# kcat/openal-soft

Hardware: AMD Instinct MI355X
Metric: mixed voices/sec @48kHz 1024-sample update, HRTF stereo; fraction of HBM roofline (higher is better)
Workload: dtype f32

## Files before the change

include/oalgpu.h:

```cpp
#ifndef OALGPU_H
#define OALGPU_H

#include <stddef.h>
#include <stdint.h>

#ifdef __cplusplus
extern "C" {
#endif
#if defined(__GNUC__)
#pragma GCC visibility push(default)
#endif

#define OALGPU_BUFFER_LINE_SIZE 1024
#define OALGPU_MAX_RESAMPLER_PADDING 48
#define OALGPU_MAX_RESAMPLER_EDGE 24
#define OALGPU_HRTF_HISTORY_LENGTH 64
#define OALGPU_HRIR_LENGTH 128
#define OALGPU_MAX_SENDS 6
#define OALGPU_MAX_OUTPUT_CHANNELS 32
#define OALGPU_MAX_AMBI_CHANNELS 25
#define OALGPU_MIXER_FRAC_BITS 16

typedef enum oalgpu_error {
    OALGPU_OK = 0,
// ... 24 lines not shown
    OALGPU_BIQUAD_HIGHSHELF, OALGPU_BIQUAD_LOWSHELF, OALGPU_BIQUAD_PEAKING, OALGPU_BIQUAD_LOWPASS,
    OALGPU_BIQUAD_HIGHPASS, OALGPU_BIQUAD_BANDPASS
} oalgpu_biquad_type;

typedef enum oalgpu_math_mode { OALGPU_MATH_EXACT = 0, OALGPU_MATH_FAST = 1 } oalgpu_math_mode;

const char *oalgpu_version(void);
const char *oalgpu_last_error(void);
int oalgpu_device_count(void);

typedef struct oalgpu_bsinc_table {
    float scaleBase, scaleRange;
    uint32_t m[16];
    uint32_t filterOffset[16];
    const float *tab;
    size_t tablen;
} oalgpu_bsinc_table;
int oalgpu_bsinc_table_get(int which , oalgpu_bsinc_table *out);
int oalgpu_cubic_table_get(int which , float *out);

typedef struct oalgpu_interp_state {
    int32_t kind;
    int32_t table;
    float sf;
    uint32_t m, l;
    uint32_t filter_offset;
} oalgpu_interp_state;
int oalgpu_prepare_resampler(int resampler, uint32_t increment, oalgpu_interp_state *out);

typedef struct oalgpu_biquad {
    float z1, z2;
    float b0, b1, b2, a1, a2;
    float tb0, tb1, tb2, ta1, ta2;
    int32_t counter;
} oalgpu_biquad;
void oalgpu_biquad_reset(oalgpu_biquad *f);
void oalgpu_biquad_set_params_from_slope(oalgpu_biquad *f, int type, float f0norm, float gain,
    float slope);

int oalgpu_resample(int device, int mode, int resampler, uint32_t increment, const float *src,
    size_t srclen, uint32_t frac, float *dst, size_t n);
int oalgpu_mix(int device, const float *in, size_t n, float *out, size_t nlines,
    float *current_gains, const float *target_gains, size_t counter, size_t outpos);
int oalgpu_mix_hrtf(int device, int mode, const float *in, float *accum, uint32_t irsize,
    const float *coeffs, const uint32_t delay[2], float gain, float gainstep, size_t n);
int oalgpu_mix_hrtf_blend(int device, int mode, const float *in, float *accum, uint32_t irsize,
    const float *oldcoeffs, const uint32_t olddelay[2], float oldgain, const float *newcoeffs,
    const uint32_t newdelay[2], float newgainstep, size_t n);
typedef struct oalgpu_splitter { float coeff, lp_z1, lp_z2, ap_z1; } oalgpu_splitter;
void oalgpu_splitter_init(oalgpu_splitter *s, float f0norm);
int oalgpu_mix_direct_hrtf(int device, int mode, float *left, float *right, const float *in,
    size_t nch, float *accum, oalgpu_splitter *splitters, const float *hfscales,
    const float *chan_coeffs, size_t irsize, size_t n);
int oalgpu_biquad_dual_process(int device, oalgpu_biquad *f0, oalgpu_biquad *f1, const float *src,
    float *dst, size_t n);

typedef struct oalgpu_context oalgpu_context;

typedef struct oalgpu_context_desc {
    int32_t  device;
    int32_t  math_mode;
    uint32_t sample_rate;
    uint32_t num_dry_channels;
    uint32_t num_real_channels;
    uint32_t num_aux_sends;
    uint32_t num_slots;
    uint32_t wet_channels;
    int32_t  hrtf;
    uint32_t max_voices;
    uint32_t max_buffers;
    uint32_t voices_per_group;
    uint32_t flags;
} oalgpu_context_desc;
#define OALGPU_CTX_FIR_VALU 1u
#define OALGPU_CTX_PROFILE  2u
#define OALGPU_CTX_STREAM_ROWS 8u
#define OALGPU_CTX_APPLY_IN_VOICE_KERNEL 16u
#define OALGPU_CTX_FUSED_REDUCE 32u
#define OALGPU_CTX_RESIDENT 64u
#define OALGPU_CTX_SLICE_LINES 128u
#define OALGPU_CTX_WAVE_PAIRS 256u
#define OALGPU_CTX_ROW_SLICES 512u
#define OALGPU_CTX_SERIAL   4u

int  oalgpu_context_create(const oalgpu_context_desc *desc, oalgpu_context **out);
void oalgpu_context_destroy(oalgpu_context *ctx);

int oalgpu_hrtf_load_mhr(oalgpu_context *ctx, const void *data, size_t size);
int oalgpu_hrtf_load_store(oalgpu_context *ctx, uint32_t sample_rate, uint32_t ir_size, const float *field_distance,
    const uint8_t *field_evcount, uint32_t num_fields, const uint16_t *elev_azcount, const uint16_t *elev_iroffset,
    uint32_t num_elevs, const float *coeffs, const uint8_t *delays, uint32_t num_irs);
typedef struct oalgpu_hrtf_info {
    uint32_t sample_rate, ir_size, num_fields, num_elevs, num_irs;
} oalgpu_hrtf_info;
int oalgpu_hrtf_info_get(oalgpu_context *ctx, oalgpu_hrtf_info *out);
int oalgpu_hrtf_raw(oalgpu_context *ctx, float *field_distance, uint8_t *field_evcount,
    uint16_t *elev_azcount, uint16_t *elev_iroffset, float *coeffs, uint8_t *delays);
int oalgpu_hrtf_get_coeffs(oalgpu_context *ctx, const float *dirs, size_t count, float *coeffs,
    uint32_t *delays);
int oalgpu_set_direct_hrtf(oalgpu_context *ctx, const float *chan_coeffs ,
    const float *hfscales, float xover_norm, uint32_t irsize);
int oalgpu_set_direct_hrtf_from_store(oalgpu_context *ctx, const float *points, const float *matrix, uint32_t num_points,
    const float *order_hf_gain, float xover_freq, uint32_t ir_size, int per_hrir_min);
int oalgpu_hrtf_parse_host(const void *mhr, size_t size, uint32_t device_rate, oalgpu_hrtf_info *info, float *coeffs, uint8_t *delays);
int oalgpu_hrtf_blend_host(const void *mhr, size_t size, uint32_t device_rate, const float *dirs, size_t count,
    uint32_t *idx, float *w, float *pass, uint32_t *delays);
int oalgpu_hrtf_build_direct_host(const void *mhr, size_t size, uint32_t device_rate, uint32_t ir_size, int per_hrir_min,
    const float *points, const float *matrix, uint32_t num_points, uint32_t num_chans, float xover_freq, const float *order_hf_gain,
    float *out_coeffs, float *out_hfscales, float *out_xover_norm, uint32_t *out_irsize);

int oalgpu_buffer_register(oalgpu_context *ctx, const void *data, int fmt_type,
    uint32_t frame_step, uint32_t sample_len, uint32_t loop_start, uint32_t loop_end);
int oalgpu_buffer_release(oalgpu_context *ctx, int buffer);
int oalgpu_buffer_info(oalgpu_context *ctx, int buffer, int32_t *live, int32_t *release_pending, uint32_t *references);

int oalgpu_buffer_channel_view(oalgpu_context *ctx, int buffer, uint32_t channel);

typedef struct oalgpu_voice_desc {
    int32_t  buffer;
    int32_t  looping;
    int32_t  position;
    uint32_t position_frac;
    uint32_t frequency;
} oalgpu_voice_desc;
int oalgpu_voice_init(oalgpu_context *ctx, uint32_t voice, const oalgpu_voice_desc *desc);
int oalgpu_context_set_nfc(oalgpu_context *ctx, float w1, const uint32_t channels_per_order[5]);
int oalgpu_voice_set_nfc(oalgpu_context *ctx, uint32_t voice, float w0);

int oalgpu_voice_set_ambi_scale(oalgpu_context *ctx, uint32_t voice, float xover_norm, float hf_scale,
    float lf_scale);

typedef struct oalgpu_filter_params {
    int32_t active;
    float gain_hf, hf_norm;
    float gain_lf, lf_norm;
} oalgpu_filter_params;

typedef struct oalgpu_voice_params {
    uint32_t step;
    int32_t  resampler;
    oalgpu_filter_params direct_filter;
    float    dry_gains[OALGPU_MAX_OUTPUT_CHANNELS];
    float    hrtf_ev, hrtf_az, hrtf_dist, hrtf_spread;
    float    hrtf_gain;
    int32_t  send_slot[OALGPU_MAX_SENDS];
    oalgpu_filter_params send_filter[OALGPU_MAX_SENDS];
    float    send_gains[OALGPU_MAX_SENDS][OALGPU_MAX_AMBI_CHANNELS];
} oalgpu_voice_params;
#define OALGPU_HRTF_KEEP_TARGET (-1.0f)
int oalgpu_voice_set_hrtf_targets(oalgpu_context *ctx, const uint32_t *voices, const float *coeffs, const uint32_t *delays,
    const float *gains, size_t count);

typedef struct oalgpu_voice_pan {
    float dir[3];
    float spread;
    float dry_gain;
    float send_gain[OALGPU_MAX_SENDS];
} oalgpu_voice_pan;
int oalgpu_context_set_ambi_map(oalgpu_context *ctx, const uint8_t *index, const float *scale);
int oalgpu_slot_set_ambi_map(oalgpu_context *ctx, uint32_t slot, const uint8_t *index, const float *scale);
int oalgpu_voice_set_pan(oalgpu_context *ctx, const uint32_t *voices, const oalgpu_voice_pan *pans, size_t count);

int oalgpu_buffer_queue_link(oalgpu_context *ctx, int buffer, int next_buffer);
int oalgpu_voice_init_queue(oalgpu_context *ctx, uint32_t voice, int first_buffer, int looping, int32_t position,
    uint32_t position_frac);
int oalgpu_voice_queue_state(oalgpu_context *ctx, uint32_t voice, int32_t *current_buffer, uint32_t *buffers_done);
// ... 182 lines not shown
    oalgpu_biquad direct_lp, direct_hp;
    float    send_current[OALGPU_MAX_SENDS][OALGPU_MAX_AMBI_CHANNELS];
    oalgpu_biquad send_lp[OALGPU_MAX_SENDS], send_hp[OALGPU_MAX_SENDS];
} oalgpu_voice_state;
int oalgpu_voice_readback(oalgpu_context *ctx, uint32_t voice, oalgpu_voice_state *out);
typedef struct oalgpu_voice_brief {
    int32_t  play_state;
    int32_t  position;
    uint32_t position_frac;
    int32_t  has_buffer;
    int32_t  fading;
    int32_t  current_buffer;
    uint32_t buffers_done;
} oalgpu_voice_brief;
int oalgpu_voices_readback(oalgpu_context *ctx, const uint32_t *voices, size_t count, oalgpu_voice_brief *out);

typedef struct oalgpu_voice_move {
    uint32_t voice;
    float hrtf_ev, hrtf_az, hrtf_dist, hrtf_spread;
    float hrtf_gain;
} oalgpu_voice_move;
int oalgpu_voice_move_async(oalgpu_context *ctx, const oalgpu_voice_move *moves, size_t count);
int oalgpu_read_output_async(oalgpu_context *ctx, uint32_t *ticket);
int oalgpu_output_wait(oalgpu_context *ctx, uint32_t ticket, float *out, size_t out_floats);

typedef struct oalgpu_voice_event {
    uint32_t voice;
    int32_t  play_state;
    int32_t  has_buffer;
    int32_t  current_buffer;
    uint32_t buffers_done;
    int32_t  position;
    uint32_t position_frac;
    int32_t  fading;
} oalgpu_voice_event;
int oalgpu_voice_events_async(oalgpu_context *ctx, uint32_t *ticket);
int oalgpu_voice_events_wait(oalgpu_context *ctx, uint32_t ticket, oalgpu_voice_event *out, size_t capacity, size_t *count);

int oalgpu_last_update_ms(oalgpu_context *ctx, float *total_ms, float *voice_kernel_ms);
int oalgpu_set_timing(oalgpu_context *ctx, int enable);
enum oalgpu_effect_kind {
    OALGPU_EFFECT_EQUALIZER = 0, OALGPU_EFFECT_MODULATOR, OALGPU_EFFECT_ECHO, OALGPU_EFFECT_DEDICATED, OALGPU_EFFECT_COMPRESSOR,
    OALGPU_EFFECT_CHORUS, OALGPU_EFFECT_DISTORTION, OALGPU_EFFECT_AUTOWAH, OALGPU_EFFECT_VMORPHER, OALGPU_EFFECT_FSHIFTER,
    OALGPU_EFFECT_PSHIFTER
};
enum oalgpu_modulator_waveform { OALGPU_MODULATOR_SINUSOID = 0, OALGPU_MODULATOR_SAWTOOTH, OALGPU_MODULATOR_SQUARE };
#define OALGPU_INVALID_CHANNEL 0xffffffffu
typedef struct oalgpu_equalizer_props {
    float low_cutoff, low_gain, mid1_center, mid1_gain, mid1_width, mid2_center, mid2_gain, mid2_width, high_cutoff, high_gain;
} oalgpu_equalizer_props;
typedef struct oalgpu_modulator_props { float frequency, high_pass_cutoff; int32_t waveform; } oalgpu_modulator_props;
typedef struct oalgpu_echo_props { float delay, lr_delay, damping, feedback, spread; } oalgpu_echo_props;
typedef struct oalgpu_compressor_props { int32_t on_off; } oalgpu_compressor_props;
enum oalgpu_chorus_waveform { OALGPU_CHORUS_SINUSOID = 0, OALGPU_CHORUS_TRIANGLE };
enum oalgpu_vmorpher_waveform { OALGPU_VMORPHER_SINUSOID = 0, OALGPU_VMORPHER_TRIANGLE, OALGPU_VMORPHER_SAWTOOTH };
enum oalgpu_fshifter_direction { OALGPU_FSHIFTER_DOWN = 0, OALGPU_FSHIFTER_UP, OALGPU_FSHIFTER_OFF };
typedef struct oalgpu_chorus_props { int32_t waveform, phase; float rate, depth, feedback, delay; } oalgpu_chorus_props;
typedef struct oalgpu_distortion_props { float edge, gain, lowpass_cutoff, eq_center, eq_bandwidth; } oalgpu_distortion_props;
typedef struct oalgpu_autowah_props { float attack_time, release_time, resonance, peak_gain; } oalgpu_autowah_props;
typedef struct oalgpu_vmorpher_props {
    float rate; int32_t phoneme_a, phoneme_b, phoneme_a_coarse_tuning, phoneme_b_coarse_tuning, waveform;
} oalgpu_vmorpher_props;
typedef struct oalgpu_fshifter_props { float frequency; int32_t left_direction, right_direction; } oalgpu_fshifter_props;
typedef struct oalgpu_pshifter_props { int32_t coarse_tune, fine_tune; } oalgpu_pshifter_props;
typedef struct oalgpu_effect oalgpu_effect;
int  oalgpu_effect_create(int device, int math_mode, int kind, uint32_t sample_rate, uint32_t num_in_channels,
    uint32_t num_out_lines, oalgpu_effect **out);
void oalgpu_effect_destroy(oalgpu_effect *effect);
int  oalgpu_effect_update(oalgpu_effect *effect, const void *props, const uint32_t *target_channels, const float *gains);
int  oalgpu_effect_process(oalgpu_effect *effect, const float *wet_in, float *out_lines, uint32_t n);
int  oalgpu_effect_set_upsampler(oalgpu_effect *effect, const float order_scales[2], float xover_norm);
int  oalgpu_slot_set_effect(oalgpu_context *ctx, uint32_t slot, oalgpu_effect *effect);

typedef struct oalgpu_converter oalgpu_converter;
int  oalgpu_converter_create(int device, int src_type, int dst_type, uint32_t channels, uint32_t src_rate,
    uint32_t dst_rate, int resampler, oalgpu_converter **out);
void oalgpu_converter_destroy(oalgpu_converter *conv);
uint32_t oalgpu_converter_available_out(const oalgpu_converter *conv, uint32_t src_frames);
int  oalgpu_converter_convert(oalgpu_converter *conv, const void **src, uint32_t *src_frames, void *dst,
    uint32_t dst_frames);

const char *oalgpu_voice_kernel_name(oalgpu_context *ctx);

typedef struct oalgpu_convolution oalgpu_convolution;
int  oalgpu_convolution_create(int device, uint32_t num_out_lines, const float *ir, uint32_t ir_len,
    oalgpu_convolution **out);
int  oalgpu_convolution_create_ex(int device, uint32_t num_out_lines, const float *ir, uint32_t ir_frames,
    uint32_t channels, uint32_t ir_rate, uint32_t device_rate, oalgpu_convolution **out);
void oalgpu_convolution_destroy(oalgpu_convolution *conv);
int  oalgpu_polyphase_resample(uint32_t src_rate, uint32_t dst_rate, const double *in, size_t n_in, double *out,
    size_t n_out);
int  oalgpu_convolution_set_target_gains(oalgpu_convolution *conv, const float *gains);
int  oalgpu_convolution_set_channel_gains(oalgpu_convolution *conv, const float *gains);
int  oalgpu_convolution_set_upsample(oalgpu_convolution *conv, const float *hf_scales, const float *lf_scales,
    float xover_norm);
int  oalgpu_convolution_process(oalgpu_convolution *conv, const float *wet_in, float *out_lines, uint32_t n);
int  oalgpu_convolution_process_device(oalgpu_convolution *conv, void *hip_stream, const float *wet_in_dev,
    float *out_lines_dev, uint32_t n);
int  oalgpu_slot_set_convolution(oalgpu_context *ctx, uint32_t slot, oalgpu_convolution *conv);

typedef struct oalgpu_reverb_props {
    float density, diffusion, gain, gain_hf, gain_lf, decay_time, decay_hf_ratio, decay_lf_ratio;
    float reflections_gain, reflections_delay, reflections_pan[3];
    float late_reverb_gain, late_reverb_delay, late_reverb_pan[3];
    float echo_time, echo_depth, modulation_time, modulation_depth, air_absorption_gain_hf;
    float hf_reference, lf_reference, room_rolloff_factor;
    int32_t decay_hf_limit;
} oalgpu_reverb_props;

typedef struct oalgpu_bq_coeffs { float b0, b1, b2, a1, a2; } oalgpu_bq_coeffs;
typedef struct oalgpu_reverb_pipeline {
    oalgpu_bq_coeffs filter_lp, filter_hp;
    uint32_t early_delay_tap[4][2];
    float    early_delay_coeff[2];
    uint32_t late_delay_tap[4][2];
    float    mix_x, mix_y;
    float    early_ap_coeff;
    uint32_t early_ap_offset[4];
    uint32_t early_offset[4];
    float    early_coeff;
    float    early_gains_target[4][OALGPU_MAX_AMBI_CHANNELS];
    uint32_t late_offset[4];
    float    late_density_gain;
    float    t60_mid_gain[4];
    oalgpu_bq_coeffs t60_hf[4], t60_lf[4];
    uint32_t mod_step;
    float    mod_depth;
    float    late_ap_coeff;
    uint32_t late_ap_offset[4];
    float    late_gains_target[4][OALGPU_MAX_AMBI_CHANNELS];
    uint32_t fade_sample_count;
} oalgpu_reverb_pipeline;
typedef struct oalgpu_reverb_params {
    int32_t pipeline_state;
    int32_t current_pipeline;
    oalgpu_reverb_pipeline pipe[2];
} oalgpu_reverb_params;
enum oalgpu_reverb_pipeline_state {
    OALGPU_REVERB_DEVICE_CLEAR = 0, OALGPU_REVERB_START_FADE = 1, OALGPU_REVERB_FADING = 2,
    OALGPU_REVERB_CLEANUP = 3, OALGPU_REVERB_NORMAL = 4
};

typedef struct oalgpu_reverb oalgpu_reverb;
int  oalgpu_reverb_create(int device, uint32_t sample_rate, uint32_t num_out_lines, oalgpu_reverb **out);
void oalgpu_reverb_destroy(oalgpu_reverb *rev);
int  oalgpu_reverb_set_upmix(oalgpu_reverb *rev, const float order_scales[2], const float *first_order_up,
    float xover_norm);
int  oalgpu_reverb_set_stream(oalgpu_reverb *rev, void *hip_stream);
int  oalgpu_reverb_set_math_mode(oalgpu_reverb *rev, int math_mode);
int  oalgpu_reverb_update(oalgpu_reverb *rev, const oalgpu_reverb_props *props, float slot_gain);
int  oalgpu_reverb_get_params(oalgpu_reverb *rev, oalgpu_reverb_params *out);
int  oalgpu_reverb_set_params(oalgpu_reverb *rev, const oalgpu_reverb_params *params);
int  oalgpu_reverb_line_lengths(oalgpu_reverb *rev, uint32_t lengths[11]);
int  oalgpu_reverb_process(oalgpu_reverb *rev, const float *wet_in, float *out_lines, uint32_t n);
int  oalgpu_reverb_process_device(oalgpu_reverb *rev, const float *wet_in_dev, float *out_lines_dev, uint32_t n);
int  oalgpu_reverb_skip(oalgpu_reverb *rev, uint32_t n);
int  oalgpu_slot_set_reverb(oalgpu_context *ctx, uint32_t slot, oalgpu_reverb *rev);

int  oalgpu_slot_set_target(oalgpu_context *ctx, uint32_t slot, int32_t target_slot);
int  oalgpu_slot_target(oalgpu_context *ctx, uint32_t slot, int32_t *target_slot);
int  oalgpu_slot_order(const int32_t *targets, uint32_t num_slots, uint32_t *order, uint32_t *depth);

#if defined(__GNUC__)
#pragma GCC visibility pop
#endif
#ifdef __cplusplus
// ... 4 lines not shown
```

openal-soft_amd/csrc/api.hip:

```cpp
#include "api_context.hpp"
namespace oalgpu {

thread_local std::string gLastError;

int Fail(int code, const std::string &msg)
{
    gLastError = msg;
    return code;
}

int UseDevice(int device)
{
    int count = 0;
    if(hipGetDeviceCount(&count) != hipSuccess || count <= 0)
        return Fail(OALGPU_ERR_NO_DEVICE, "no HIP device available (the product has no CPU path)");
    if(device < 0 || device >= count) return Fail(OALGPU_ERR_INVALID, "device ordinal out of range");
    HIP_TRY(hipSetDevice(device));
    ParkResidentContexts(device);
    return OALGPU_OK;
}

}

int UseCtx(oalgpu_context *c)
// ... 143 lines not shown
    L.firMfma = (desc->flags & OALGPU_CTX_FIR_VALU) ? 0u : 1u;
    c->serialOnly = (desc->flags & OALGPU_CTX_SERIAL) != 0;
    c->res.enabled = (desc->flags & OALGPU_CTX_RESIDENT) != 0 && !(desc->flags & (OALGPU_CTX_PROFILE | OALGPU_CTX_SERIAL));
    c->useWave = WaveKernelApplies(c->exact, L);
    if(c->useWave)
    {
        L.waveVoices = desc->voices_per_group ? std::max<uint32_t>(1u, (desc->voices_per_group + 3u) / 4u)
            : std::max<uint32_t>(1u, (desc->max_voices + 2047u) / 2048u);
        L.numGroups = std::max<uint32_t>(1u, WaveKernelGroups(L));
    }
    const TableBlob &blob = Blob();
    HIP_TRY(c->tables.alloc(blob.data.size())); HIP_TRY(c->tables.upload(blob.data.data(), blob.data.size()));
    L.tables = c->tables.p;
    HIP_TRY(c->buffers.alloc(std::max<uint32_t>(desc->max_buffers, 1u))); HIP_TRY(c->buffers.zero());
    L.buffers = c->buffers.p;
    c->buf.reset(desc->max_buffers, desc->max_voices);
    c->cbOfVoice.assign(std::max<uint32_t>(desc->max_voices, 1u), -1);

    const size_t nv = desc->max_voices;
    HIP_TRY(c->ctl.alloc(nv)); HIP_TRY(c->ctl.zero()); L.ctl = c->ctl.p;
    HIP_TRY(c->prev.alloc(nv * kMaxPad)); HIP_TRY(c->prev.zero()); L.prev = c->prev.p;
    HIP_TRY(c->dfilt.alloc(nv * 2)); HIP_TRY(c->dfilt.zero()); L.dfilt = c->dfilt.p;
    HIP_TRY(c->hist.alloc(nv * kHist)); HIP_TRY(c->hist.zero()); L.hist = c->hist.p;
    HIP_TRY(c->gainCur.alloc(nv * L.numDry)); HIP_TRY(c->gainCur.zero()); L.gainCur = c->gainCur.p;
    HIP_TRY(c->gainTgt.alloc(nv * L.numDry)); HIP_TRY(c->gainTgt.zero()); L.gainTgt = c->gainTgt.p;
    HIP_TRY(c->sfilt.alloc(nv * L.numSends * 2)); HIP_TRY(c->sfilt.zero()); L.sfilt = c->sfilt.p;
    HIP_TRY(c->sendCur.alloc(nv * L.numSends * L.wetChannels)); HIP_TRY(c->sendCur.zero()); L.sendCur = c->sendCur.p;
    HIP_TRY(c->sendTgt.alloc(nv * L.numSends * L.wetChannels)); HIP_TRY(c->sendTgt.zero()); L.sendTgt = c->sendTgt.p;
    HIP_TRY(c->ambi.alloc(nv)); HIP_TRY(c->ambi.zero()); L.ambi = c->ambi.p;
    HIP_TRY(c->startDelay.alloc(nv)); HIP_TRY(c->startDelay.zero()); L.startDelay = c->startDelay.p;
    {
        std::vector<AmbiMapEntry> ident(std::max<size_t>(L.numDry, size_t{L.numSlots} * L.wetChannels) + 1);
        for(size_t i = 0; i < ident.size(); ++i) ident[i] = AmbiMapEntry{uint32_t(i < OALGPU_MAX_AMBI_CHANNELS ? i : 0), 1.0f};
        HIP_TRY(c->dryMap.alloc(L.numDry)); HIP_TRY(c->dryMap.upload(ident.data(), L.numDry));
        HIP_TRY(c->wetMaps.alloc(size_t{L.numSlots} * L.wetChannels));
        for(uint32_t s = 0; s < L.numSlots; ++s)
            HIP_TRY(hipMemcpy(c->wetMaps.p + size_t{s} * L.wetChannels, ident.data(), L.wetChannels * sizeof(AmbiMapEntry), hipMemcpyHostToDevice));
    }
    HIP_TRY(c->queueDone.alloc(nv)); HIP_TRY(c->queueDone.zero()); L.queueDone = c->queueDone.p;
    L.numLineGroups = L.numGroups;
    c->groupsAllocated = L.numGroups;
    if(c->useWave && L.hrtf && L.firMfma && !(desc->flags & OALGPU_CTX_WAVE_PAIRS))
    {
        const uint32_t w = Wave16WavesFor(desc->max_voices, DeviceComputeUnits(desc->device));
        c->groupsAllocated = std::max<uint32_t>(c->groupsAllocated, (desc->max_voices + w - 1u) / w);
    }
    L.streams = nullptr; L.lineGains = nullptr; L.lineStride = 0; L.streamsPerVoice = 0;
    L.nfc = nullptr; L.nfcOrders = 0;
    L.hrirs = nullptr;
    for(uint32_t &n : L.chansPerOrder) n = 0;
    L.accLines = 0;
    L.wave16 = 0;
    L.rows8 = 0; L.rowsVpg = 0;
    if(c->useWave && !(desc->flags & OALGPU_CTX_STREAM_ROWS))
    {
        L.accLines = WaveKernelAccLines(L);
        if(!L.accLines && RowsKernelApplies(L))
            L.rows8 = 1;
    }
    if(c->useWave && (!L.hrtf || L.numSends))
    {
        L.lineStride = L.mixLines <= 8 ? 8u : (L.mixLines <= 16 ? 16u : 32u);
        L.streamsPerVoice = 2u + L.numSends;
    }
    if(c->useWave && (!L.hrtf || L.numSends) && !L.accLines && !L.rows8) { if(int rc = AllocStreamRows(c.get())) return rc; }
    const size_t groups = c->groupsAllocated;
    HIP_TRY(c->partLines.alloc(groups * L.mixLines * kLine)); L.partLines = c->partLines.p;
    HIP_TRY(c->partLines2.alloc(c->useWave && (L.streams || L.accLines || L.rows8) ? groups * L.mixLines * kLine : 0));
    c->partLinesBuf[0] = c->partLines.p; c->partLinesBuf[1] = c->partLines2.p;
    HIP_TRY(c->partHrtf.alloc(L.hrtf ? groups * (kLine + kHrirLen) * 2 : 0)); L.partHrtf = c->partHrtf.p;
    HIP_TRY(c->partHrtf2.alloc(c->useWave && L.hrtf ? groups * (kLine + kHrirLen) * 2 : 0));
    c->partHrtfBuf[0] = c->partHrtf.p; c->partHrtfBuf[1] = c->partHrtf2.p;
    HIP_TRY(c->bus.alloc(BusFloats(L))); HIP_TRY(c->bus.zero()); L.bus = c->bus.p;
    if(desc->flags & OALGPU_CTX_PROFILE)
    {
        HIP_TRY(c->phaseTimes.alloc(nv * 16)); HIP_TRY(c->phaseTimes.zero());
        c->prof.times = c->phaseTimes.p;
    }
    L.hrtfOld = nullptr; L.hrtfTgt = nullptr;

    HIP_TRY(c->dSplit.alloc(L.numDry)); HIP_TRY(c->dSplit.zero());
    HIP_TRY(c->dSplit2.alloc(L.numDry)); HIP_TRY(c->dSplit2.zero());
    HIP_TRY(c->carryBuf.alloc(size_t{kLine + kHrirLen} * 2)); HIP_TRY(c->carryBuf.zero());
    HIP_TRY(c->postArrived.alloc(1)); HIP_TRY(c->postArrived.zero());
    HIP_TRY(c->dHfScale.alloc(L.numDry)); HIP_TRY(c->dHfScale.zero());
    HIP_TRY(c->dCoeffs.alloc(size_t{L.numDry} * kHrirLen * 2)); HIP_TRY(c->dCoeffs.zero());
    HIP_TRY(c->dTemp.alloc(size_t{L.numDry} * kLine + (kLine + kHrirLen) * 2));
    if(L.rows8) SetRowsGroups(c.get());
    *out = c.release();
    return OALGPU_OK;
}

void oalgpu_context_destroy(oalgpu_context *ctx)
{
    if(!ctx) return;
    (void)UseDevice(ctx->desc.device);
    if(ctx->attachedTo || !ctx->attached.empty()) DetachForDestroy(ctx);
    if(ctx->res.pendingBlock) { ctx->res.pendingBlock->heldBy = nullptr; ctx->res.pendingBlock = nullptr; }
    (void)FlushPendingMix(ctx);
    (void)hipStreamSynchronize(ctx->stream);
    if(ctx->res.reduceStream) (void)hipStreamSynchronize(ctx->res.reduceStream);
    if(ctx->postStream) (void)hipStreamSynchronize(ctx->postStream);
    delete ctx->comm;
    for(auto &cb : ctx->cbVoices)
        for(int k = 0; k < 2; ++k)
        {
            if(cb.pinned[k]) (void)hipHostFree(cb.pinned[k]);
            if(cb.copied[k]) (void)hipEventDestroy(cb.copied[k]);
        }
    delete ctx;
}

int AllocStreamRows(oalgpu_context *c)
{
    DeviceLayout &L = c->L;
    const size_t nv = L.numVoices;
    HIP_TRY(c->streams.alloc(nv * L.streamsPerVoice * kLine)); HIP_TRY(c->streams.zero()); L.streams = c->streams.p;
    HIP_TRY(c->lineGains.alloc(nv * L.streamsPerVoice * LineBlockDwords(L.lineStride))); HIP_TRY(c->lineGains.zero());
    L.lineGains = c->lineGains.p;
    return OALGPU_OK;
}

const float *CarrySource(oalgpu_context *c, bool carry)
{
    const float *src = nullptr;
    if(carry && c->L.hrtf) src = c->carryInBuf ? c->carryBuf.p : c->L.bus + BusAccumOffset(c->L);
    c->carryInBuf = false;
    return src;
}

static void SplitterRunPowers(float coeff, uint32_t seg, float out[4])
{
    const float ap = coeff, lp = coeff * 0.5f + 0.5f;
    float st[3][3] = {{1.0f, 0.0f, 0.0f}, {0.0f, 1.0f, 0.0f}, {0.0f, 0.0f, 1.0f}};
    for(uint32_t i = 0; i < seg; ++i)
        for(auto &v : st)
        {
            const float d0 = (0.0f - v[0]) * lp;
            const float lpY0 = v[0] + d0;
            v[0] = std::fmaf(d0, lp, lpY0);
            const float d1 = (lpY0 - v[1]) * lp;
            const float lpY1 = v[1] + d1;
            v[1] = lpY1 + d1;
            const float apY = std::fmaf(0.0f, ap, v[2]);
            v[2] = std::fmaf(-apY, ap, 0.0f);
        }
    out[0] = st[0][0]; out[1] = st[0][1]; out[2] = st[1][1]; out[3] = st[2][2];
}

int PostDirectHrtfFused(oalgpu_context *c, hipStream_t s, uint32_t samples_to_do, hipEvent_t evDone, bool resident)
{
    const DeviceLayout &L = c->L;
    float *left = L.bus + size_t{L.numDry} * kLine;
    SplitterState *spIn = c->dSplitCur ? c->dSplit2.p : c->dSplit.p, *spOut = c->dSplitCur ? c->dSplit.p : c->dSplit2.p;
    const uint32_t postEpoch = c->postEpoch + L.numDry;
    const uint32_t seg = ((samples_to_do + 63u) / 64u) | 1u;
    if(c->runPowerSeg != seg) { SplitterRunPowers(c->dSplitCoeff, seg, c->runPower); c->runPowerSeg = seg; }
    const uint32_t slot = c->outNext % oalgpu_context::kIoSlots;
    const bool ring = c->outRing && c->outFlags;
    const uint32_t outTarget = c->outArrivedTotal + PostResidentFirGroups();
    const PostHrtfCall call{left, left + kLine, L.bus, L.numDry, L.bus + BusAccumOffset(L), c->carryBuf.p, spIn, spOut, c->dHfScale.p, c->dCoeffs.p,
        c->dIrSize, samples_to_do, c->dTemp.p, c->postArrived.p, postEpoch, c->runPower, evDone, ring ? c->outHost[slot] : nullptr,
        ring ? c->outFlags + size_t{slot} * 16 : nullptr, c->outSeq + 1u};
    auto &R = c->res;
    if(resident)
    {
        c->reduceHeld = false;
        LaunchPostResident(s, call, R.counters.p, R.hostFlags, (R.posts + 1u) * R.redGroups, (R.posts + 1u) * R.firGroups, R.posts + 1u);
        HIP_TRY(hipGetLastError());
        ++R.posts;
    }
    else if(c->reduceHeld)
    {
        c->reduceHeld = false;
        if(!c->reducedCount.p) { HIP_TRY(c->reducedCount.alloc(1)); HIP_TRY(c->reducedCount.zero()); }
        const uint32_t reducedEpoch = c->reducedEpoch + ReducePostReduceGroups(c->heldL);
        LaunchReducePostFused(s, call, c->heldL, CarrySource(c, c->carryAccum && L.hrtf), c->outArrived.p, outTarget, c->reducedCount.p, reducedEpoch);
        HIP_TRY(hipGetLastError());
        c->reducedEpoch = reducedEpoch;
        if(ring) c->outArrivedTotal = outTarget;
    }
    else
    {
        LaunchPostDirectHrtfFused(s, call, c->outArrived.p, outTarget);
        HIP_TRY(hipGetLastError());
        if(ring) c->outArrivedTotal = outTarget;
    }
    c->postEpoch = postEpoch;
    if(ring) c->outSlotSeq[slot] = ++c->outSeq;
    c->outRingWritten = ring;
    c->dSplitCur ^= 1u;
    c->carryInBuf = true;
    return OALGPU_OK;
}

int JoinPost(oalgpu_context *c)
{
    if(!c->postPending) return OALGPU_OK;
    HIP_TRY(hipStreamWaitEvent(c->stream, c->lastPostEvent ? c->lastPostEvent : c->evPostDone, 0));
    c->postPending = false;
    return OALGPU_OK;
}

static int RefuseWithoutHrtfData(const oalgpu_context *c)
{
    if(c->L.hrtf && !c->hrtfLoaded) return Fail(OALGPU_ERR_NO_HRTF, "HRTF context without a data set");
    return OALGPU_OK;
}

enum : uint32_t { kNeedsFast = 1u, kNeedsHrtfData = 2u };
static int BeginUpdate(oalgpu_context *c, const char *who, uint32_t samples_to_do, uint32_t needs = 0u)
{
    if(!c || samples_to_do == 0 || samples_to_do > kLine) return Fail(OALGPU_ERR_INVALID, "samples_to_do must be 1..1024");
    if((needs & kNeedsFast) && !(c->useWave && c->ownStream))
        return Fail(OALGPU_ERR_INVALID, std::string(who) + ": needs a FAST context (wavefront kernel) on its own streams");
    if(int rc = RefuseAttached(c, who)) return rc;
    return (needs & kNeedsHrtfData) ? RefuseWithoutHrtfData(c) : OALGPU_OK;
}

static int BeforeVoices(oalgpu_context *c, uint32_t samples_to_do)
{
    if(!c->cbVoices.empty()) { if(int rc = ServiceCallbacks(c, samples_to_do)) return rc; }
    if(!c->attached.empty()) { if(int rc = MixAttached(c, samples_to_do)) return rc; }
    c->outRingWritten = false;
    return OALGPU_OK;
}

static int EndTimedUpdate(oalgpu_context *c, hipStream_t s)
{
    if(!c->timing) return OALGPU_OK;
    HIP_TRY(hipEventRecord(c->evEnd, s));
    c->timed = true;
    return OALGPU_OK;
}

int oalgpu_mix_voices(oalgpu_context *c, uint32_t samples_to_do)
{
    if(int rc = BeginUpdate(c, "oalgpu_mix_voices", samples_to_do)) return rc;
    return MixVoicesSerial(c, samples_to_do);
}

int MixVoicesSerial(oalgpu_context *c, uint32_t samples_to_do)
{
    if(int rc = RefuseWithoutHrtfData(c)) return rc;
    if(int rc = UseCtx(c)) return rc;
    if(int rc = FlushInits(c)) return rc;
    if(int rc = JoinPost(c)) return rc;
    if(int rc = BeforeVoices(c, samples_to_do)) return rc;
    if(c->useWave)
        HIP_TRY(LaunchVoiceWave(c->stream, c->L, samples_to_do, c->profArg(), c->timing ? c->evStart : nullptr, c->timing ? c->evVoice : nullptr));
    else
    {
        if(c->timing) HIP_TRY(hipEventRecord(c->evStart, c->stream));
        HIP_TRY(LaunchVoiceMix(c->stream, c->exact, c->L, samples_to_do, c->carryAccum));
        if(c->timing) HIP_TRY(hipEventRecord(c->evVoice, c->stream));
    }
    if(c->attachedTo && c->attachedTo->mergeInFlight) HIP_TRY(hipStreamWaitEvent(c->stream, c->attachedTo->evMerged, 0));
    LaunchBusReduce(c->stream, c->L, samples_to_do, CarrySource(c, c->useWave && c->carryAccum));
    HIP_TRY(hipGetLastError());
    if(int rc = CommReduceBus(c, c->stream)) return rc;
    return EndTimedUpdate(c, c->stream);
}

int oalgpu_post_process(oalgpu_context *c, uint32_t samples_to_do)
{
    if(int rc = BeginUpdate(c, "oalgpu_post_process", samples_to_do)) return rc;
    if(int rc = UseCtx(c)) return rc;
    if(int rc = JoinPost(c)) return rc;
    if(!c->attached.empty()) { if(int rc = MergeAttached(c, c->stream, samples_to_do)) return rc; }
    if(int rc = RunEffects(c, c->stream, samples_to_do)) return rc;
    if(!c->L.hrtf)
    {
        if(int rc = RunSpeakerPost(c, c->stream, samples_to_do)) return rc;
        return EndTimedUpdate(c, c->stream);
    }
    const DeviceLayout &L = c->L;
    if(L.numReal < 2) return Fail(OALGPU_ERR_INVALID, "HRTF post-process needs two real output lines");
    float *left = L.bus + size_t{L.numDry} * kLine;
    float *right = left + kLine;
    SplitterState *spCur = c->dSplitCur ? c->dSplit2.p : c->dSplit.p;
    if(c->exact)
        LaunchMixDirectHrtf(c->stream, true, left, right, L.bus, L.numDry, L.bus + BusAccumOffset(L), spCur,
            c->dHfScale.p, c->dCoeffs.p, c->dIrSize, samples_to_do, c->dTemp.p);
    else if(c->useWave) { if(int rc = PostDirectHrtfFused(c, c->stream, samples_to_do, nullptr)) return rc; }
    else
        LaunchPostDirectHrtfFast(c->stream, left, right, L.bus, L.numDry, L.bus + BusAccumOffset(L), spCur,
            c->dHfScale.p, c->dCoeffs.p, c->dIrSize, samples_to_do, c->dTemp.p);
    HIP_TRY(hipGetLastError());
    if(int rc = RunLimiter(c, c->stream, samples_to_do)) return rc;
    return EndTimedUpdate(c, c->stream);
}

static int RunMixUpdate(oalgpu_context *c, uint32_t samples_to_do, int post_process, oalgpu_param_block *next);

int oalgpu_mix_update(oalgpu_context *c, uint32_t samples_to_do, int post_process)
{
    if(int rc = BeginUpdate(c, "oalgpu_mix_update", samples_to_do, kNeedsHrtfData)) return rc;
    if(c->res.cooldown) --c->res.cooldown;
    else if(ResidentWanted(c, post_process))
    {
        const int rc = ResidentSubmit(c, samples_to_do);
        if(rc <= 0) return rc;
    }
    if(int rc = UseCtx(c)) return rc;
    if(c->useWave && c->ownStream && !c->serialOnly && !c->timing && (c->desc.flags & OALGPU_CTX_APPLY_IN_VOICE_KERNEL) && WaveKernelAppliesRecords(c->L)
        && !(c->res.enabled && !c->res.failed && !c->res.cooldown))
    {
        c->pendingMix.active = true; c->pendingMix.samples = samples_to_do; c->pendingMix.post = post_process;
        return OALGPU_OK;
    }
    return RunMixUpdate(c, samples_to_do, post_process, nullptr);
}

int BeginSetter(oalgpu_context *c, const char *who)
{
    if(!c) return Fail(OALGPU_ERR_INVALID, std::string(who) + ": null context");
    if(int rc = FlushPendingMix(c)) return rc;
    return c->res.pendingBlock ? UseCtx(c) : OALGPU_OK;
}

int FlushPendingMix(oalgpu_context *c, oalgpu_param_block *next)
{
    if(c->attachedTo) { if(int rc = FlushPendingMix(c->attachedTo)) return rc; }
    if(!c->pendingMix.active) return OALGPU_OK;
    c->pendingMix.active = false;
    return RunMixUpdate(c, c->pendingMix.samples, c->pendingMix.post, next);
}

static int RunMixUpdate(oalgpu_context *c, uint32_t samples_to_do, int post_process, oalgpu_param_block *next)
{
    c->nextRecs = next ? next->recs.p : nullptr;
    c->nextMap = next ? next->voiceToRec.p : nullptr;
    c->nextRows = next ? next->rows.p : nullptr;
    struct Clear { oalgpu_context *c; ~Clear() { c->nextRecs = nullptr; c->nextMap = nullptr; c->nextRows = nullptr; } } clear{c};
    if(!(c->useWave && c->ownStream) || c->serialOnly)
    {
        if(int rc = oalgpu_mix_voices(c, samples_to_do)) return rc;
        if(post_process && c->commRank == 0) return oalgpu_post_process(c, samples_to_do);
        return OALGPU_OK;
    }
    c->fuseReduce = post_process && !c->comm && c->L.hrtf && c->L.numSlots == 0 && c->L.numReal >= 2 && !c->timing
        && (c->desc.flags & OALGPU_CTX_FUSED_REDUCE) && c->attached.empty();
    const int rcv = oalgpu_mix_voices_overlapped(c, samples_to_do);
    c->fuseReduce = false;
    if(rcv) { c->reduceHeld = false; return rcv; }
    return oalgpu_post_process_overlapped(c, samples_to_do, post_process && c->commRank == 0);
}

int oalgpu_mix_update_run(oalgpu_context *c, oalgpu_param_block *const *param_blocks, uint32_t count, uint32_t samples_to_do,
    int post_process)
{
    if(!c || count == 0) return Fail(OALGPU_ERR_INVALID, "oalgpu_mix_update_run: bad arguments");
    if(int rc = RefuseAttached(c, "oalgpu_mix_update_run")) return rc;
    for(uint32_t i = 0; i < count; ++i)
    {
        if(param_blocks && param_blocks[i]) { if(int rc = oalgpu_param_block_apply(c, param_blocks[i])) return rc; }
        if(int rc = oalgpu_mix_update(c, samples_to_do, post_process)) return rc;
    }
    return OALGPU_OK;
}

int oalgpu_mix_voices_overlapped(oalgpu_context *c, uint32_t samples_to_do)
{
    if(int rc = BeginUpdate(c, "oalgpu_mix_voices_overlapped", samples_to_do, kNeedsFast | kNeedsHrtfData)) return rc;
    if(int rc = UseCtx(c)) return rc;
    if(int rc = FlushInits(c)) return rc;
    if(int rc = BeforeVoices(c, samples_to_do)) return rc;
    const uint32_t p = c->parity;
    DeviceLayout L = c->L;
    L.partHrtf = c->partHrtfBuf[p];
    if(L.streams || L.accLines || L.rows8) L.partLines = c->partLinesBuf[p];
    if(c->reduceUpdate[p] > c->updatesKnownDone)
    {
        const hipError_t q = hipEventQuery(c->evReduceDone[p]);
        if(q == hipErrorNotReady) HIP_TRY(hipStreamWaitEvent(c->stream, c->evReduceDone[p], 0));
        else HIP_TRY(q);
    }
    c->reduceUpdate[p] = ++c->updatesSubmitted;
    HIP_TRY(LaunchVoiceWave(c->stream, L, samples_to_do, c->profArg(), c->timing ? c->evStart : nullptr, c->timing ? c->evVoice : c->evVoiceDone[p],
        c->nextRecs, c->nextMap, c->nextRows));
    if(c->timing) HIP_TRY(hipEventRecord(c->evVoiceDone[p], c->stream));
    HIP_TRY(hipStreamWaitEvent(c->postStream, c->evVoiceDone[p], 0));
    if(c->fuseReduce)
    {
        c->reduceHeld = true; c->heldL = L; c->heldParity = p;
        c->parity = p ^ 1u;
        return OALGPU_OK;
    }
    LaunchBusReduce(c->postStream, L, samples_to_do, CarrySource(c, c->carryAccum && L.hrtf), true, c->evReduceDone[p]);
    HIP_TRY(hipGetLastError());
    if(int rc = CommReduceBus(c, c->postStream)) return rc;
    c->parity = p ^ 1u;
    return OALGPU_OK;
}

void *oalgpu_post_stream(oalgpu_context *c) { return c ? static_cast<void*>(c->postStream) : nullptr; }

int oalgpu_post_process_overlapped(oalgpu_context *c, uint32_t samples_to_do, int post_process)
{
    if(int rc = BeginUpdate(c, "oalgpu_post_process_overlapped", samples_to_do, kNeedsFast)) return rc;
    if(post_process && c->L.hrtf && c->L.numReal < 2) return Fail(OALGPU_ERR_INVALID, "HRTF post-process needs two real output lines");
    if(int rc = UseCtx(c)) return rc;
    const DeviceLayout &L = c->L;
    bool postDoneBound = false;
    if(post_process && !c->attached.empty()) { if(int rc = MergeAttached(c, c->postStream, samples_to_do)) return rc; }
    if(post_process) { if(int rc = RunEffects(c, c->postStream, samples_to_do)) return rc; }
    if(post_process && L.hrtf)
    {
        hipEvent_t ev = c->reduceHeld ? c->evReduceDone[c->heldParity] : ((c->timing || c->limOn) ? nullptr : c->evPostDone);
        c->lastPostEvent = (ev && !c->limOn) ? ev : c->evPostDone;
        if(int rc = PostDirectHrtfFused(c, c->postStream, samples_to_do, ev)) return rc;
        postDoneBound = ev != nullptr && !c->limOn;
        if(int rc = RunLimiter(c, c->postStream, samples_to_do)) return rc;
    }
    else
    {
        c->lastPostEvent = c->evPostDone;
        if(post_process) { if(int rc = RunSpeakerPost(c, c->postStream, samples_to_do)) return rc; }
    }
    if(int rc = EndTimedUpdate(c, c->postStream)) return rc;
    if(!postDoneBound) HIP_TRY(hipEventRecord(c->evPostDone, c->postStream));
    c->postPending = true;
    return OALGPU_OK;
}

int oalgpu_sync(oalgpu_context *c)
{
    if(!c) return Fail(OALGPU_ERR_INVALID, "null argument");
    if(int rc = UseCtx(c)) return rc;
    HIP_TRY(hipStreamSynchronize(c->stream));
    if(c->res.reduceStream) HIP_TRY(hipStreamSynchronize(c->res.reduceStream));
    if(c->postStream) HIP_TRY(hipStreamSynchronize(c->postStream));
    c->postPending = false;
    c->updatesKnownDone = c->updatesSubmitted;
    for(oalgpu_context *a : c->attached)
    {
        HIP_TRY(hipStreamSynchronize(a->stream));
        if(a->postStream) HIP_TRY(hipStreamSynchronize(a->postStream));
        a->postPending = false;
        a->updatesKnownDone = a->updatesSubmitted;
    }
    c->mergeInFlight = false;
    if(c->res.ready) { ResidentCollectTimes(c, true); if(int rc = ResidentCheckError(c)) return rc; }
    return OALGPU_OK;
}

int oalgpu_set_timing(oalgpu_context *c, int enable)
{
    if(int rc = BeginSetter(c, "oalgpu_set_timing")) return rc;
    c->timing = enable != 0;
    c->timed = false;
    return OALGPU_OK;
}

int oalgpu_last_update_ms(oalgpu_context *c, float *total_ms, float *voice_kernel_ms)
{
    if(!c || !c->timed) return Fail(OALGPU_ERR_INVALID, "no timed update (call oalgpu_set_timing first)");
    if(int rc = oalgpu_sync(c)) return rc;
    if(total_ms) HIP_TRY(hipEventElapsedTime(total_ms, c->evStart, c->evEnd));
    if(voice_kernel_ms) HIP_TRY(hipEventElapsedTime(voice_kernel_ms, c->evStart, c->evVoice));
    return OALGPU_OK;
}

#ifdef OALGPU_MEASUREMENT
int oalgpu_debug_set_ablate(oalgpu_context *c, uint32_t mask)
{
    if(!c || !c->phaseTimes.p) return Fail(OALGPU_ERR_INVALID, "not an OALGPU_CTX_PROFILE context");
    c->prof.ablate = mask;
    return OALGPU_OK;
}

int oalgpu_debug_phase_times(oalgpu_context *c, unsigned long long *out)
{
    if(!c || !out || !c->phaseTimes.p) return Fail(OALGPU_ERR_INVALID, "phase times were not enabled");
    if(int rc = oalgpu_sync(c)) return rc;
    HIP_TRY(hipMemcpy(out, c->phaseTimes.p, size_t{c->L.numVoices} * 8 * sizeof(unsigned long long), hipMemcpyDeviceToHost));
    return OALGPU_OK;
}

int oalgpu_debug_wave_times(oalgpu_context *c, unsigned long long *out, uint32_t *waves)
{
    if(!c || !out || !waves || !c->phaseTimes.p) return Fail(OALGPU_ERR_INVALID, "phase times were not enabled");
    if(int rc = oalgpu_sync(c)) return rc;
    HIP_TRY(hipMemcpy(out, c->phaseTimes.p + size_t{c->L.numVoices} * 8, size_t{c->L.numVoices} * 8 * sizeof(unsigned long long), hipMemcpyDeviceToHost));
    *waves = WaveKernelGroups(c->L) * 4u;
    return OALGPU_OK;
}

#endif

const char *oalgpu_voice_kernel_name(oalgpu_context *c)
{
    if(!c) return "";
    if(c->useWave) return WaveKernelName(c->L);
// ... 10 lines not shown
```

openal-soft_amd/csrc/api_attach.hip:

```cpp
#include "api_context.hpp"

int RefuseAttached(const oalgpu_context *c, const char *who)
{
    if(!c->attachedTo) return OALGPU_OK;
    return Fail(OALGPU_ERR_INVALID, std::string(who) + ": the context is attached (oalgpu_context_attach): its device context updates it");
}

int MixAttached(oalgpu_context *c, uint32_t samples_to_do)
{
    for(oalgpu_context *a : c->attached) { if(int rc = MixVoicesSerial(a, samples_to_do)) return rc; }
    return OALGPU_OK;
}

int MergeAttached(oalgpu_context *c, hipStream_t s, uint32_t samples_to_do)
{
    for(oalgpu_context *a : c->attached)
    {
        if(int rc = RunEffects(a, a->stream, samples_to_do)) return rc;
        HIP_TRY(hipEventRecord(a->evBusFinal, a->stream));
        HIP_TRY(hipStreamWaitEvent(s, a->evBusFinal, 0));
    }
    LaunchBusMerge(s, c->mergeHeads.p, c->mergeRows.p, c->mergeLines, samples_to_do);
    HIP_TRY(hipGetLastError());
    HIP_TRY(hipEventRecord(c->evMerged, s));
    c->mergeInFlight = true;
    return OALGPU_OK;
}

static int RebuildMergeTable(oalgpu_context *d)
{
    const uint32_t lines = d->L.numDry + d->L.numReal;
    std::vector<BusMergeHead> heads;
    std::vector<BusMergeRow> rows;
    std::vector<int32_t> last(lines, -1);
    for(uint32_t line = 0; line < lines; ++line)
        for(const oalgpu_context *a : d->attached)
            for(size_t i = 0; i < a->attachMap.size(); ++i)
            {
                if(a->attachMap[i] != int32_t(line)) continue;
                const int32_t r = int32_t(rows.size());
                rows.push_back(BusMergeRow{a->L.bus + i * kLine, -1, 0u});
                if(last[line] < 0) heads.push_back(BusMergeHead{d->L.bus + size_t{line} * kLine, r, 0u});
                else rows[size_t(last[line])].next = r;
                last[line] = r;
            }
    DevBuf<BusMergeHead> newHeads;
    DevBuf<BusMergeRow> newRows;
    if(!heads.empty())
    {
        HIP_TRY(newHeads.alloc(heads.size())); HIP_TRY(newHeads.upload(heads.data(), heads.size()));
        HIP_TRY(newRows.alloc(rows.size())); HIP_TRY(newRows.upload(rows.data(), rows.size()));
    }
    std::swap(d->mergeHeads.p, newHeads.p); std::swap(d->mergeHeads.n, newHeads.n);
    std::swap(d->mergeRows.p, newRows.p); std::swap(d->mergeRows.n, newRows.n);
    d->mergeLines = uint32_t(heads.size());
    return OALGPU_OK;
}

static void Unlink(oalgpu_context *a)
{
    oalgpu_context *d = a->attachedTo;
    d->attached.erase(std::remove(d->attached.begin(), d->attached.end(), a), d->attached.end());
    a->attachedTo = nullptr;
    a->attachMap.clear();
    d->mergeInFlight = false;
}

int oalgpu_context_attach(oalgpu_context *d, oalgpu_context *a, const int32_t *line_map)
{
    const std::string w = "oalgpu_context_attach: ";
    if(!d || !a || !line_map) return Fail(OALGPU_ERR_INVALID, w + "null argument");
    if(d == a) return Fail(OALGPU_ERR_INVALID, w + "a context cannot be attached to itself");
    if(a->attachedTo) return Fail(OALGPU_ERR_INVALID, w + "the context is already attached");
    if(d->attachedTo) return Fail(OALGPU_ERR_INVALID, w + "the device context is itself attached (no nesting)");
    if(!a->attached.empty()) return Fail(OALGPU_ERR_INVALID, w + "the context has attached contexts of its own (no nesting)");
    if(d->desc.device != a->desc.device) return Fail(OALGPU_ERR_INVALID, w + "the contexts are on different devices");
    if(d->desc.sample_rate != a->desc.sample_rate) return Fail(OALGPU_ERR_INVALID, w + "the contexts have different sample rates");
    if(a->L.hrtf) return Fail(OALGPU_ERR_INVALID, w + "an HRTF context cannot be attached (HRTF voices belong to the device context)");
    if(a->post != PostKind::None) return Fail(OALGPU_ERR_INVALID, w + "the context has a post-process installed (the device context post-processes)");
    if(a->limOn) return Fail(OALGPU_ERR_INVALID, w + "the context has an output limiter (the device context limits)");
    if(a->distLines) return Fail(OALGPU_ERR_INVALID, w + "the context has distance compensation (the device context compensates)");
    if(a->outType != OALGPU_OUT_F32 || a->ditherDepth > 0.0f)
        return Fail(OALGPU_ERR_INVALID, w + "the context has an output conversion (oalgpu_set_output: the device context converts)");
    if(d->comm || a->comm) return Fail(OALGPU_ERR_INVALID, w + "a context with a collective (oalgpu_comm_init) takes and is no attachment");
    if(!a->ownStream) return Fail(OALGPU_ERR_INVALID, w + "the context is on a caller-owned stream (oalgpu_set_stream)");
    const uint32_t srcLines = a->L.numDry + a->L.numReal, dstLines = d->L.numDry + d->L.numReal;
    for(uint32_t i = 0; i < srcLines; ++i)
        if(line_map[i] < -1 || line_map[i] >= int32_t(dstLines))
            return Fail(OALGPU_ERR_INVALID, w + "map entry " + std::to_string(i) + " is out of range (-1 .. " + std::to_string(dstLines - 1u) + ")");
    if(int rc = oalgpu_sync(d)) return rc;
    if(int rc = oalgpu_sync(a)) return rc;
    if(!a->evBusFinal) HIP_TRY(hipEventCreateWithFlags(&a->evBusFinal, hipEventDisableTiming | hipEventDisableSystemFence));
    if(!d->evMerged) HIP_TRY(hipEventCreateWithFlags(&d->evMerged, hipEventDisableTiming | hipEventDisableSystemFence));
    a->attachMap.assign(line_map, line_map + srcLines);
    a->attachedTo = d;
    d->attached.push_back(a);
    if(int rc = RebuildMergeTable(d))
    {
        Unlink(a);
        (void)RebuildMergeTable(d);
        return rc;
    }
    return OALGPU_OK;
}

int oalgpu_context_detach(oalgpu_context *a)
{
    if(!a) return Fail(OALGPU_ERR_INVALID, "oalgpu_context_detach: null argument");
    oalgpu_context *d = a->attachedTo;
    if(!d) return Fail(OALGPU_ERR_INVALID, "oalgpu_context_detach: the context is not attached");
    if(int rc = oalgpu_sync(d)) return rc;
    Unlink(a);
    return RebuildMergeTable(d);
}

void DetachForDestroy(oalgpu_context *ctx)
{
    if(oalgpu_context *d = ctx->attachedTo)
    {
        (void)oalgpu_sync(d);
        Unlink(ctx);
        (void)RebuildMergeTable(d);
    }
    if(!ctx->attached.empty())
    {
        (void)oalgpu_sync(ctx);
        while(!ctx->attached.empty()) Unlink(ctx->attached.back());
        ctx->mergeLines = 0;
    }
}
```

openal-soft_amd/csrc/api_comm.hip:

```cpp
#include "api_context.hpp"

namespace {
struct RcclApi {
    ncclResult_t (*getUniqueId)(ncclUniqueId*) = nullptr;
    ncclResult_t (*commInitRank)(ncclComm_t*, int, ncclUniqueId, int) = nullptr;
    ncclResult_t (*commDestroy)(ncclComm_t) = nullptr;
    ncclResult_t (*reduce)(const void*, void*, size_t, ncclDataType_t, ncclRedOp_t, int, ncclComm_t, hipStream_t) = nullptr;
    const char *(*getErrorString)(ncclResult_t) = nullptr;
    ncclResult_t (*commCount)(const ncclComm_t, int*) = nullptr;
    bool ok = false;
    std::string why;
};

RcclApi &Rccl()
{
    static RcclApi api = []
    {
        RcclApi a;
        void *h = nullptr;
        if(dlsym(RTLD_DEFAULT, "ncclCommInitRank")) h = RTLD_DEFAULT;
        else
        {
            for(const char *name : {"librccl.so.1", "librccl.so", "/opt/rocm/lib/librccl.so.1"})
                if((h = dlopen(name, RTLD_NOW | RTLD_LOCAL))) break;
// ... 96 lines not shown
    }
    static void Gather(void *p)
    {
        HostTransport *t = static_cast<HostTransport*>(p);
        const uint64_t q = t->executed++;
        float *dst = t->pinned[q % kSlots];
        for(int r = 1; r < t->world; ++r)
        {
            if(!WaitFor([&] { return t->hdr->produced[r].load(std::memory_order_acquire) > q; }, t->hdr->failed))
            { std::memset(dst, 0, t->floats * sizeof(float)); return; }
            const float *src = t->slot(r, q);
            if(r == 1) std::memcpy(dst, src, t->floats * sizeof(float));
            else for(size_t i = 0; i < t->floats; ++i) dst[i] += src[i];
        }
        t->hdr->consumed.store(q + 1, std::memory_order_release);
    }
    int reduceToRoot(oalgpu_context *c, hipStream_t s) override
    {
        if(hdr->failed.load()) return Fail(OALGPU_ERR_HIP, "host transport: a rank timed out waiting for its peers");
        const uint64_t q = submitted++;
        if(rank != 0)
        {
            HIP_TRY(hipMemcpyAsync(pinned[q % kSlots], c->L.bus, bytes, hipMemcpyDeviceToHost, s));
            HIP_TRY(hipLaunchHostFunc(s, Produce, this));
            return OALGPU_OK;
        }
        if(world == 1) return OALGPU_OK;
        HIP_TRY(hipLaunchHostFunc(s, Gather, this));
        HIP_TRY(hipMemcpyAsync(devSum.p, pinned[q % kSlots], bytes, hipMemcpyHostToDevice, s));
        hipLaunchKernelGGL(AddBusKernel, dim3(uint32_t((floats + 255) / 256)), dim3(256), 0, s, c->L.bus, devSum.p, uint32_t(floats));
        HIP_TRY(hipGetLastError());
        return OALGPU_OK;
    }
    ~HostTransport() override
    {
        for(float *p : pinned) if(p) (void)hipHostFree(p);
        if(hdr) munmap(hdr, sizeof(Header) + size_t(world) * kSlots * bytes);
        if(fd >= 0) close(fd);
        if(rank == 0 && !name.empty()) shm_unlink(name.c_str());
    }
};

}

int CommReduceBus(oalgpu_context *c, hipStream_t s)
{
    if(!c->comm) return OALGPU_OK;
    return c->comm->reduceToRoot(c, s);
}

extern "C" {

int oalgpu_comm_unique_id(void *out, size_t size)
{
    if(!out || size < sizeof(ncclUniqueId)) return Fail(OALGPU_ERR_INVALID, "oalgpu_comm_unique_id: 128 bytes needed");
    RcclApi &a = Rccl();
    if(!a.ok) return Fail(OALGPU_ERR_NO_DEVICE, a.why);
    ncclUniqueId id;
    const ncclResult_t r = a.getUniqueId(&id);
    if(r != ncclSuccess) return FailRccl("ncclGetUniqueId", r);
    std::memcpy(out, &id, sizeof(id));
    return OALGPU_OK;
}

int oalgpu_comm_init(oalgpu_context *c, const void *unique_id, size_t size, int rank, int world)
{
    if(!c || !unique_id || size < sizeof(ncclUniqueId) || world < 1 || rank < 0 || rank >= world)
        return Fail(OALGPU_ERR_INVALID, "oalgpu_comm_init: bad arguments");
    if(c->comm) return Fail(OALGPU_ERR_INVALID, "oalgpu_comm_init: the context already has a communicator");
    if(c->attachedTo || !c->attached.empty())
        return Fail(OALGPU_ERR_INVALID, "oalgpu_comm_init: not on a context that has, or is, an attachment (oalgpu_context_attach)");
    if(!c->cbVoices.empty()) return Fail(OALGPU_ERR_INVALID, "oalgpu_comm_init: not on a context with callback sources");
    RcclApi &a = Rccl();
    if(!a.ok) return Fail(OALGPU_ERR_NO_DEVICE, a.why);
    if(int rc = UseCtx(c)) return rc;
    if(int rc = oalgpu_sync(c)) return rc;
    ncclUniqueId id;
    std::memcpy(&id, unique_id, sizeof(id));
    auto t = std::make_unique<RcclTransport>();
    const ncclResult_t r = a.commInitRank(&t->comm, world, id, rank);
    if(r != ncclSuccess) return FailRccl("ncclCommInitRank", r);
    c->comm = t.release(); c->commRank = rank; c->commWorld = world;
    c->carryAccum = rank == 0;
    return OALGPU_OK;
}

int oalgpu_comm_init_host(oalgpu_context *c, const char *name, int rank, int world)
{
    if(!c || !name || name[0] != '/' || world < 1 || world > int(HostTransport::kMaxWorld) || rank < 0 || rank >= world)
        return Fail(OALGPU_ERR_INVALID, "oalgpu_comm_init_host: bad arguments");
    if(c->comm) return Fail(OALGPU_ERR_INVALID, "oalgpu_comm_init_host: the context already has a communicator");
    if(c->attachedTo || !c->attached.empty())
        return Fail(OALGPU_ERR_INVALID, "oalgpu_comm_init_host: not on a context that has, or is, an attachment (oalgpu_context_attach)");
    if(!c->cbVoices.empty()) return Fail(OALGPU_ERR_INVALID, "oalgpu_comm_init_host: not on a context with callback sources");
    if(int rc = UseCtx(c)) return rc;
    if(int rc = oalgpu_sync(c)) return rc;
    auto t = std::make_unique<HostTransport>();
    t->name = name; t->rank = rank; t->world = world;
    t->floats = BusFloats(c->L); t->bytes = t->floats * sizeof(float);
    const size_t total = sizeof(HostTransport::Header) + size_t(world) * HostTransport::kSlots * t->bytes;
    using clk = std::chrono::steady_clock;
    const auto deadline = clk::now() + std::chrono::seconds(60);
    for(float *&p : t->pinned) HIP_TRY(hipHostMalloc(reinterpret_cast<void**>(&p), t->bytes, hipHostMallocDefault));
    if(rank == 0)
    {
        HIP_TRY(t->devSum.alloc(t->floats));
        shm_unlink(name);
        t->fd = shm_open(name, O_CREAT | O_EXCL | O_RDWR, 0600);
        if(t->fd < 0 || ftruncate(t->fd, off_t(total)) != 0) return Fail(OALGPU_ERR_HIP, std::string("shm_open/ftruncate ") + name + " failed");
        void *m = mmap(nullptr, total, PROT_READ | PROT_WRITE, MAP_SHARED, t->fd, 0);
        if(m == MAP_FAILED) return Fail(OALGPU_ERR_HIP, "mmap of the shared segment failed");
        t->hdr = static_cast<HostTransport::Header*>(m);
        t->ring = reinterpret_cast<float*>(static_cast<char*>(m) + sizeof(HostTransport::Header));
        t->hdr->world = uint32_t(world); t->hdr->floats = uint32_t(t->floats);
        t->hdr->magic.store(0x0a16b05u, std::memory_order_release);
        for(int r = 1; r < world; ++r)
        {
            uint64_t tok = 0;
            while((tok = t->hdr->hello[r].load(std::memory_order_acquire)) == 0)
            {
                if(clk::now() > deadline) return Fail(OALGPU_ERR_HIP, "oalgpu_comm_init_host: a rank did not attach within 60 s");
                std::this_thread::sleep_for(std::chrono::milliseconds(1));
            }
            t->hdr->ack[r].store(tok, std::memory_order_release);
        }
    }
    else
    {
        const uint64_t token = ((uint64_t(getpid()) << 32) ^ uint64_t(clk::now().time_since_epoch().count()) ^ (uint64_t(rank) << 56)) | 1ull;
        bool attached = false;
        std::string why = "rank 0's segment did not appear";
        while(!attached && clk::now() < deadline)
        {
            t->fd = shm_open(name, O_RDWR, 0600);
            struct stat st{};
            if(t->fd >= 0 && (fstat(t->fd, &st) != 0 || size_t(st.st_size) < total)) { close(t->fd); t->fd = -1; }
            if(t->fd < 0) { std::this_thread::sleep_for(std::chrono::milliseconds(10)); continue; }
            void *m = mmap(nullptr, total, PROT_READ | PROT_WRITE, MAP_SHARED, t->fd, 0);
            if(m == MAP_FAILED) return Fail(OALGPU_ERR_HIP, "mmap of the shared segment failed");
            auto *hdr = static_cast<HostTransport::Header*>(m);
            const auto patience = clk::now() + std::chrono::seconds(3);
            bool said = false;
            while(clk::now() < patience && clk::now() < deadline)
            {
                if(hdr->magic.load(std::memory_order_acquire) == 0x0a16b05u)
                {
                    if(hdr->world != uint32_t(world) || hdr->floats != uint32_t(t->floats)) { why = "the ranks' contexts differ (world size or bus block)"; break; }
                    if(!said) { hdr->hello[rank].store(token, std::memory_order_release); said = true; }
                    if(hdr->ack[rank].load(std::memory_order_acquire) == token) { attached = true; break; }
                }
                std::this_thread::sleep_for(std::chrono::milliseconds(1));
            }
            if(attached)
            {
                t->hdr = hdr;
                t->ring = reinterpret_cast<float*>(static_cast<char*>(m) + sizeof(HostTransport::Header));
            }
            else
            {
                munmap(m, total); close(t->fd); t->fd = -1;
                if(why.find("differ") != std::string::npos) return Fail(OALGPU_ERR_INVALID, "oalgpu_comm_init_host: " + why);
                why = "no live rank 0 answered on the segment";
            }
        }
        if(!attached) return Fail(OALGPU_ERR_HIP, std::string("shm_open ") + name + ": " + why);
    }
    c->comm = t.release(); c->commRank = rank; c->commWorld = world;
    c->carryAccum = rank == 0;
    return OALGPU_OK;
}

int oalgpu_comm_info(oalgpu_context *c, int *rank, int *world, int *transport_ranks, char *kind, size_t kind_size)
{
    if(!c) return Fail(OALGPU_ERR_INVALID, "null argument");
    if(rank) *rank = c->commRank;
    if(world) *world = c->commWorld;
    if(transport_ranks) *transport_ranks = c->comm ? c->comm->ranks() : 1;
    if(kind && kind_size) { std::snprintf(kind, kind_size, "%s", c->comm ? c->comm->kind() : "none"); }
    return OALGPU_OK;
}

int oalgpu_comm_destroy(oalgpu_context *c)
{
    if(!c) return Fail(OALGPU_ERR_INVALID, "null argument");
    if(!c->comm) return OALGPU_OK;
    if(int rc = oalgpu_sync(c)) return rc;
    delete c->comm;
    c->comm = nullptr; c->commRank = 0; c->commWorld = 1; c->carryAccum = true;
    return OALGPU_OK;
}

}
```

openal-soft_amd/csrc/api_context.hpp:

```cpp
#pragma once
#include "../../include/oalgpu.h"
#ifdef OALGPU_MEASUREMENT
#include "../../tools/measure/oalgpu_measure.h"
#endif

#include <hip/hip_runtime.h>
#include <hip/hip_ext.h>
#include <rccl/rccl.h>
#include <dlfcn.h>
#include <fcntl.h>
#include <sys/mman.h>
#include <sys/stat.h>
#include <unistd.h>

#include <algorithm>
#include <atomic>
#include <chrono>
#include <functional>
#include <thread>
#include <cstdio>
#include <cstdlib>
#include <cstring>
#include <memory>
#include <mutex>
// ... 109 lines not shown
    HrtfStoreDev hrtfDev{};
    HrtfData hrtfHost;
    bool hrtfLoaded{false};
    uint32_t hrtfGeneration{0};
    bool carryAccum{true};
    bool useWave{false};
    uint32_t groupsAllocated{0};
    std::vector<EffectSlot> slots;
    std::vector<uint32_t> slotOrder;
    DevBuf<uint32_t> reverbTicket;

    DevBuf<float> tables;
    DevBuf<BufferItem> buffers;
    DevBuf<uint32_t> startDelay;
    DevBuf<uint32_t> queueDone;
    BufferTable buf;
    DevBuf<VoiceCtl> ctl;
    DevBuf<float> prev, hrtfOld, hrtfTgt, hist, gainCur, gainTgt, sendCur, sendTgt;
    DevBuf<BiquadSlot> dfilt, sfilt;
    DevBuf<float> partLines, partLines2, partHrtf, partHrtf2, bus, streams;
    DevBuf<uint32_t> lineGains;
    DevBuf<AmbiScaleState> ambi;
    DevBuf<NfcState> nfc;
    NfcDesign nfcDevice{};
    DevBuf<unsigned long long> phaseTimes;
    WaveProf prof{nullptr, 0u};
    const WaveProf *profArg() const { return prof.times ? &prof : nullptr; }
    DevBuf<AmbiMapEntry> dryMap, wetMaps;
    DevBuf<PanRecord> panRecs;
    std::vector<VoiceCtl> ctlHost;
    std::vector<uint32_t> doneHost;
    DevBuf<TargetRecord> tgtRecs;
    DevBuf<float> tgtCoeffs;
    bool serialOnly{false};
    struct BusTransport *comm{nullptr};
    int commRank{0}, commWorld{1};
    oalgpu_context *attachedTo{nullptr};
    std::vector<int32_t> attachMap;
    hipEvent_t evBusFinal{nullptr};
    std::vector<oalgpu_context*> attached;
    DevBuf<BusMergeHead> mergeHeads;
    DevBuf<BusMergeRow> mergeRows;
    uint32_t mergeLines{0};
    hipEvent_t evMerged{nullptr};
    bool mergeInFlight{false};
    PostKind post{PostKind::None};
    bool decDual{false};
    uint32_t decOut{0};
    DevBuf<float> decGainsHf, decGainsLf, decBands;
    DevBuf<SplitterState> decSplit;
    int outType{6};
    float ditherDepth{0.0f};
    uint32_t ditherSeed{22222};
    bool limOn{false};
    LimiterConsts lim{};
    DevBuf<float> limState;
    int encQuality{-1};
    DevBuf<float> encTaps, encState;
    uint32_t stabLeft{0}, stabRight{0}, stabCenter{0};
    StabilizerConsts stab{};
    DevBuf<float> stabState;
    uint32_t cfLeft{0}, cfRight{0};
    CrossfeedConsts cf{};
    DevBuf<float> cfState;
    uint32_t distLines{0};
    DevBuf<uint32_t> distDelays;
    DevBuf<float> distGains, distHist;
    DevBuf<unsigned char> pcm;
    DevBuf<float> hFieldDist, hCoeffs;
    DevBuf<uint8_t> hEvCount, hDelays;
    DevBuf<uint16_t> hAzCount, hIrOffset;
    DevBuf<SplitterState> dSplit, dSplit2;
    uint32_t dSplitCur{0};
    DevBuf<float> carryBuf;
    float dSplitCoeff{0.0f};
    float runPower[4]{1.0f, 0.0f, 1.0f, 1.0f};
    uint32_t runPowerSeg{0};
    DevBuf<uint32_t> postArrived;
    uint32_t postEpoch{0};
    const ParamRecord *nextRecs{nullptr};
    const int32_t *nextMap{nullptr};
    const float *nextRows{nullptr};
    bool carryInBuf{false};
    DevBuf<float> dHfScale, dCoeffs, dTemp;
    uint32_t dIrSize{0};
    bool directSet{false};
    DevBuf<ParamRecord> paramDev;
    std::vector<ParamRecord> paramHost;
    DevBuf<VoiceInitRecord> initDev;
    std::vector<VoiceInitRecord> initPending;
    oalgpu_listener_params listener{{1.0f, 0.0f, 0.0f, 0.0f, 0.0f, 1.0f, 0.0f, 0.0f, 0.0f, 0.0f, 1.0f, 0.0f, 0.0f, 0.0f, 0.0f, 1.0f}, {}, {},
        1.0f, 1.0f, 0.99426f, 1.0f, 343.3f, 0, OALGPU_DISTANCE_DISABLE, 1.0f, 1.0f, {1.0f, 1.0f, 1.0f}};
    std::vector<oalgpu_slot_environment> slotEnvHost;
    DevBuf<oalgpu_slot_environment> slotEnv;
    DevBuf<ResamplerConsts> rsConsts;
    std::vector<uint32_t> voiceFreq;
    DevBuf<SourceRecord> srcDev;
    std::vector<SourceRecord> srcHost;
    std::vector<uint32_t> srcVoices;
    DevBuf<ChannelSourceRecord> chanDev;
    std::vector<ChannelSourceRecord> chanHost;
    struct CbVoice {
        uint32_t voice{0}; int32_t buffer{-1}; uint32_t frameBytes{4}, capacityFrames{0};
        oalgpu_callback_fn fn{nullptr}; void *user{nullptr};
        std::vector<char> data;
        uint32_t numBlocks{0}, blockOffset{0};
        bool stopped{false};
        int32_t position{0}; uint32_t frac{0}, step{0};
        int state{OALGPU_VOICE_PLAYING}; bool hasBuffer{true};
        char *pinned[2]{nullptr, nullptr}; hipEvent_t copied[2]{nullptr, nullptr}; uint32_t slot{0};
        size_t allocBytes{0};
        bool retired{false};
    };
    std::vector<CbVoice> cbVoices;
    std::vector<int32_t> cbOfVoice;

    struct ResidentState {
        bool enabled{false};
        bool ready{false}, failed{false};
        bool running{false};
        hipStream_t reduceStream{nullptr};
        ResidentDoor *door{nullptr};
        bool doorInBar{false};
        DevBuf<uint32_t> counters;
        uint32_t *hostFlags{nullptr};
        DevBuf<float> part;
        size_t setFloats{0};
        uint32_t next{0};
        uint32_t endSeq{0};
        uint32_t launches{0}, startedTotal{0};
        uint32_t launchBase{0};
        uint32_t shortRuns{0}, cooldown{0};
        uint32_t shortRun{32};
        uint32_t awaitStarted{0};
        uint32_t maxUpdates{4096};
        uint32_t setUses[kResidentSets]{};
        uint32_t posts{0};
        uint32_t firGroups{0}, redGroups{0}, groupsPerCu{0};
        oalgpu_param_block *pendingBlock{nullptr};
        hipEvent_t copyPending{nullptr};
        static constexpr uint32_t kEv = 4;
        hipEvent_t evStart[kEv]{}, evStop[kEv]{};
        uint32_t evFirst[kEv]{}, evLast[kEv]{};
        bool evOpen[kEv]{};
        bool timeLaunches{false};
        double kernelMs{0.0};
        uint64_t kernelUpdates{0}, kernelLaunches{0}, parks{0};
    } res;

    ~oalgpu_context()
    {
        for(int h = 0; buf.inRange(h); ++h) (void)hipFree(buf.at(h).storage);
        for(uint32_t k = 0; k < kIoSlots; ++k)
        {
            if(panHost[k]) (void)(panInBar ? hipFree(panHost[k]) : hipHostFree(panHost[k]));
            if(outHost[k]) (void)hipHostFree(outHost[k]);
            if(evHost[k]) (void)hipHostFree(evHost[k]);
            if(evDone[k]) (void)hipEventDestroy(evDone[k]);
            for(hipEvent_t e : {panApplied[k], outDone[k]}) if(e) (void)hipEventDestroy(e);
        }
        if(outFlags) (void)hipHostFree(outFlags);
        if(res.door) (void)(res.doorInBar ? hipFree(res.door) : hipHostFree(res.door));
        if(res.hostFlags) (void)hipHostFree(res.hostFlags);
        for(uint32_t k = 0; k < ResidentState::kEv; ++k)
            for(hipEvent_t e : {res.evStart[k], res.evStop[k]}) if(e) (void)hipEventDestroy(e);
        if(res.reduceStream) (void)hipStreamDestroy(res.reduceStream);
        for(hipEvent_t e : {evBusFinal, evMerged}) if(e) (void)hipEventDestroy(e);
        if(evStart) (void)hipEventDestroy(evStart);
        if(evVoice) (void)hipEventDestroy(evVoice);
        if(evEnd) (void)hipEventDestroy(evEnd);
        for(hipEvent_t e : {evVoiceDone[0], evVoiceDone[1], evReduceDone[0], evReduceDone[1], evPostDone})
            if(e) (void)hipEventDestroy(e);
        if(postStream) (void)hipStreamDestroy(postStream);
        if(stream && ownStream) (void)hipStreamDestroy(stream);
    }
};

struct oalgpu_param_block {
    DevBuf<ParamRecord> recs;
    uint32_t count{0};
    int device{0};
    uint32_t hrtfGeneration{0};
    DevBuf<int32_t> voiceToRec;
    uint32_t mapVoices{0};
    DevBuf<float> rows;
    std::vector<std::pair<uint32_t, uint32_t>> cbSteps;
    oalgpu_context *heldBy{nullptr};
};

struct BusTransport {
    virtual ~BusTransport() = default;
    virtual int reduceToRoot(oalgpu_context *c, hipStream_t s) = 0;
    virtual int ranks() const = 0;
    virtual const char *kind() const = 0;
};

namespace oalgpu { extern thread_local std::string gLastError; }

int FlushPendingMix(oalgpu_context *c, struct oalgpu_param_block *next = nullptr);
int UseCtx(oalgpu_context *c);
int MixVoicesSerial(oalgpu_context *c, uint32_t samples_to_do);
const float *CarrySource(oalgpu_context *c, bool carry);
int PostDirectHrtfFused(oalgpu_context *c, hipStream_t s, uint32_t samples_to_do, hipEvent_t evDone, bool resident = false);
int RebalanceWaveGroups(oalgpu_context *c);
namespace oalgpu { void ParkResidentContexts(int device); }
bool ResidentWanted(const oalgpu_context *c, int post_process);
int FlushResidentBlock(oalgpu_context *c);
int ResidentSubmit(oalgpu_context *c, uint32_t samples_to_do);
void ResidentCollectTimes(oalgpu_context *c, bool all);
int ResidentCheckError(oalgpu_context *c);
int RefuseAttached(const oalgpu_context *c, const char *who);
int MixAttached(oalgpu_context *c, uint32_t samples_to_do);
int MergeAttached(oalgpu_context *c, hipStream_t s, uint32_t samples_to_do);
void DetachForDestroy(oalgpu_context *ctx);
int RunEffects(oalgpu_context *c, hipStream_t s, uint32_t samples_to_do);
uint32_t AttachedReverbs(const oalgpu_context *c);
int UseCtxResident(oalgpu_context *c);
void RetireCallbackVoice(oalgpu_context *c, uint32_t voice);
void NoteCallbackSteps(oalgpu_context *c, const uint32_t *voices, const oalgpu_voice_params *params, size_t count);
int FlushInits(oalgpu_context *c);
int AllocStreamRows(oalgpu_context *c);
uint32_t DeviceComputeUnits(int device);
int JoinPost(oalgpu_context *c);
int BeginSetter(oalgpu_context *c, const char *who);
int RunSpeakerPost(oalgpu_context *c, hipStream_t s, uint32_t samplesToDo);
int RunLimiter(oalgpu_context *c, hipStream_t s, uint32_t samplesToDo);
bool RingEligible(const oalgpu_context *c);
inline float *RealOut(const oalgpu_context *c) { return c->L.numReal ? c->L.bus + size_t{c->L.numDry} * kLine : c->L.bus; }
inline uint32_t RealOutLines(const oalgpu_context *c) { return c->L.numReal ? c->L.numReal : c->L.numDry; }
bool HostStoresReachDevice(oalgpu_context *c);
int RegisterBuffer(oalgpu_context *c, void *storage, BufferItem item, uint32_t loopLen, int parent);
void FreeStorage(const std::vector<void*> &freed);
inline bool VoiceOk(const oalgpu_context *c, uint32_t voice) { return c && voice < c->L.numVoices; }
int BeginVoiceCall(oalgpu_context *c, bool argsOk = true, const char *who = "", bool sync = false);
void PendStart(oalgpu_context *c, const VoiceInitRecord &rec);
int FinishParamBlock(oalgpu_context *c, struct oalgpu_param_block *b, const uint32_t *voices, size_t count);
oalgpu::HrtfStoreDev HostStoreView(const oalgpu::HrtfData &h);
int ServiceCallbacks(oalgpu_context *c, uint32_t samplesToDo);
int CommReduceBus(oalgpu_context *c, hipStream_t s);
```

openal-soft_amd/csrc/api_output.hip:

```cpp
#include "api_context.hpp"

static size_t OutputLineFloats(const oalgpu_context *c) { return size_t{RealOutLines(c)} * kLine; }

bool RingEligible(const oalgpu_context *c)
{
    return c->L.hrtf && c->L.numReal == 2 && c->useWave && OutputLineFloats(c) == size_t{2} * kLine && !c->limOn;
}

int oalgpu_read_output_async(oalgpu_context *c, uint32_t *ticket)
{
    if(!c || !ticket) return Fail(OALGPU_ERR_INVALID, "null argument");
    const size_t floats = OutputLineFloats(c);
    if(int rc = (c->outFloats != floats) ? UseCtx(c) : UseCtxResident(c)) return rc;
    if(c->outFloats != floats)
    {
        for(uint32_t k = 0; k < oalgpu_context::kIoSlots; ++k)
        {
            if(c->outHost[k]) { HIP_TRY(hipHostFree(c->outHost[k])); c->outHost[k] = nullptr; }
            HIP_TRY(hipHostMalloc(reinterpret_cast<void**>(&c->outHost[k]), floats * sizeof(float), hipHostMallocDefault));
            if(!c->outDone[k]) HIP_TRY(hipEventCreateWithFlags(&c->outDone[k], hipEventDisableTiming));
        }
        c->outFloats = floats;
        if(!c->outFlags)
        {
// ... 60 lines not shown
    constexpr uint32_t slots = oalgpu_context::kIoSlots;
    if(!c->evHost[0])
    {
        for(uint32_t k = 0; k < slots; ++k)
        {
            HIP_TRY(hipHostMalloc(reinterpret_cast<void**>(&c->evHost[k]), (4u + size_t{oalgpu_context::kEvCap} * 8u) * sizeof(uint32_t), hipHostMallocDefault));
            HIP_TRY(hipEventCreateWithFlags(&c->evDone[k], hipEventDisableTiming));
        }
        HIP_TRY(c->evSnapshot.alloc(size_t{c->L.numVoices} * 3)); HIP_TRY(c->evSnapshot.zero());
        HIP_TRY(c->evCounters.alloc(2)); HIP_TRY(c->evCounters.zero());
        std::vector<uint32_t> init(size_t{c->L.numVoices} * 3, 0u);
        for(uint32_t v = 0; v < c->L.numVoices; ++v) { init[size_t{v} * 3 + 0] = uint32_t(OALGPU_VOICE_STOPPED); init[size_t{v} * 3 + 1] = 0xffffffffu; }
        HIP_TRY(hipMemcpyAsync(c->evSnapshot.p, init.data(), init.size() * sizeof(uint32_t), hipMemcpyHostToDevice, c->stream));
        HIP_TRY(hipStreamSynchronize(c->stream));
    }
    const uint32_t slot = c->evNext % slots;
    LaunchVoiceEvents(c->stream, c->L, c->evSnapshot.p, c->evHost[slot], oalgpu_context::kEvCap, c->evCounters.p);
    HIP_TRY(hipGetLastError());
    HIP_TRY(hipEventRecord(c->evDone[slot], c->stream));
    *ticket = c->evNext++;
    return OALGPU_OK;
}

int oalgpu_voice_events_wait(oalgpu_context *c, uint32_t ticket, oalgpu_voice_event *out, size_t capacity, size_t *count)
{
    if(!c || !count || (!out && capacity)) return Fail(OALGPU_ERR_INVALID, "null argument");
    if(ticket >= c->evNext || c->evNext - ticket > oalgpu_context::kIoSlots)
        return Fail(OALGPU_ERR_INVALID, "oalgpu_voice_events_wait: the ticket's slot was reused (four tickets may be outstanding)");
    if(int rc = UseCtxResident(c)) return rc;
    const uint32_t slot = ticket % oalgpu_context::kIoSlots;
    HIP_TRY(hipEventSynchronize(c->evDone[slot]));
    const uint32_t *h = c->evHost[slot];
    const uint32_t n = h[0];
    *count = n;
    if(n > oalgpu_context::kEvCap || n > capacity)
        return Fail(OALGPU_ERR_CAPACITY, "oalgpu_voice_events_wait: " + std::to_string(n) + " changes, more than the report holds (read the voices back: oalgpu_voices_readback)");
    for(uint32_t i = 0; i < n; ++i)
    {
        const uint32_t *e = h + 4u + size_t{i} * 8u;
        out[i] = oalgpu_voice_event{e[0], int32_t(e[1]), int32_t(e[2]) >= 0 ? 1 : 0, int32_t(e[2]), e[3], int32_t(e[4]), e[5], int32_t(e[6])};
        if(e[0] < c->L.numVoices) c->buf.noteQueueDone(e[0], e[3]);
    }
    return OALGPU_OK;
}

int oalgpu_set_stream(oalgpu_context *c, void *hip_stream)
{
    if(!c) return Fail(OALGPU_ERR_INVALID, "null argument");
    if(hip_stream && c->attachedTo)
        return Fail(OALGPU_ERR_INVALID, "oalgpu_set_stream: an attached context (oalgpu_context_attach) stays on its own streams");
    if(int rc = UseCtx(c)) return rc;
    HIP_TRY(hipStreamSynchronize(c->stream));
    if(c->postStream) HIP_TRY(hipStreamSynchronize(c->postStream));
    c->postPending = false;
    if(c->ownStream && c->stream) { (void)hipStreamDestroy(c->stream); c->stream = nullptr; }
    if(hip_stream) { c->stream = static_cast<hipStream_t>(hip_stream); c->ownStream = false; }
    else
    {
        int prioLeast = 0, prioGreatest = 0;
        HIP_TRY(hipDeviceGetStreamPriorityRange(&prioLeast, &prioGreatest));
        HIP_TRY(hipStreamCreateWithPriority(&c->stream, hipStreamDefault, prioGreatest));
        c->ownStream = true;
    }
    return OALGPU_OK;
}


int oalgpu_read_dry(oalgpu_context *c, float *out)
{
    if(!c || !out) return Fail(OALGPU_ERR_INVALID, "null argument");
    if(int rc = oalgpu_sync(c)) return rc;
    HIP_TRY(hipMemcpy(out, c->L.bus, BusWetOffset(c->L) * sizeof(float), hipMemcpyDeviceToHost));
    return OALGPU_OK;
}

int oalgpu_set_output(oalgpu_context *c, int sample_type, float dither_depth, uint32_t dither_seed)
{
    if(int rc = BeginSetter(c, "oalgpu_set_output")) return rc;
    if(sample_type < OALGPU_OUT_I8 || sample_type > OALGPU_OUT_F32 || dither_depth < 0.0f)
        return Fail(OALGPU_ERR_INVALID, "oalgpu_set_output: bad arguments");
    if(c->attachedTo && (sample_type != OALGPU_OUT_F32 || dither_depth > 0.0f))
        return Fail(OALGPU_ERR_INVALID, "oalgpu_set_output: the context is attached (oalgpu_context_attach): its device context has the post stage");
    c->outType = sample_type; c->ditherDepth = dither_depth; c->ditherSeed = dither_seed;
    return OALGPU_OK;
}

int oalgpu_read_output(oalgpu_context *c, void *out, uint32_t samples_to_do, uint32_t frame_step)
{
    static const size_t bytesPer[7] = {1, 1, 2, 2, 4, 4, 4};
    if(!c || !out || samples_to_do == 0 || samples_to_do > kLine || frame_step == 0 || frame_step > 64)
        return Fail(OALGPU_ERR_INVALID, "oalgpu_read_output: bad arguments");
    if(int rc = UseCtx(c)) return rc;
    if(int rc = JoinPost(c)) return rc;
    float *lines = RealOut(c);
    const uint32_t all = RealOutLines(c);
    const uint32_t nlines = std::min(all, frame_step);
    if(c->ditherDepth > 0.0f)
    {
        LaunchDither(c->stream, lines, all, samples_to_do, c->ditherDepth, c->ditherSeed);
        c->ditherSeed = DitherAdvanceSeed(c->ditherSeed, all * samples_to_do * 2u);
    }
    const size_t nbytes = size_t{samples_to_do} * frame_step * bytesPer[c->outType];
    if(c->pcm.n < nbytes) HIP_TRY(c->pcm.alloc(size_t{kLine} * 64 * 4));
    LaunchWriteSamples(c->stream, c->outType, lines, nlines, samples_to_do, frame_step, c->pcm.p);
    HIP_TRY(hipGetLastError());
    HIP_TRY(hipMemcpyAsync(out, c->pcm.p, nbytes, hipMemcpyDeviceToHost, c->stream));
    HIP_TRY(hipStreamSynchronize(c->stream));
    return OALGPU_OK;
}

int oalgpu_read_wet(oalgpu_context *c, uint32_t slot, float *out)
{
    if(!c || !out || slot >= c->L.numSlots) return Fail(OALGPU_ERR_INVALID, "bad slot");
    if(int rc = oalgpu_sync(c)) return rc;
    const size_t n = size_t{c->L.wetChannels} * kLine;
    HIP_TRY(hipMemcpy(out, c->L.bus + BusWetOffset(c->L) + slot * n, n * sizeof(float), hipMemcpyDeviceToHost));
    return OALGPU_OK;
}

int oalgpu_read_hrtf_accum(oalgpu_context *c, float *out)
{
    if(!c || !out) return Fail(OALGPU_ERR_INVALID, "null argument");
    if(int rc = oalgpu_sync(c)) return rc;
    HIP_TRY(hipMemcpy(out, c->carryInBuf ? c->carryBuf.p : c->L.bus + BusAccumOffset(c->L), size_t{kLine + kHrirLen} * 2 * sizeof(float), hipMemcpyDeviceToHost));
    return OALGPU_OK;
}

int oalgpu_bus_device_ptr(oalgpu_context *c, void **ptr, size_t *nfloats, void **hip_stream)
{
    if(int rc = BeginSetter(c, "oalgpu_bus_device_ptr")) return rc;
    if(!ptr || !nfloats) return Fail(OALGPU_ERR_INVALID, "null argument");
    *ptr = c->L.bus;
    *nfloats = BusFloats(c->L);
    if(hip_stream)
        *hip_stream = (c->useWave && c->ownStream && !c->serialOnly && c->postStream) ? c->postStream : c->stream;
    return OALGPU_OK;
}

int oalgpu_voice_readback(oalgpu_context *c, uint32_t v, oalgpu_voice_state *out)
{
    if(int rc = BeginVoiceCall(c, VoiceOk(c, v) && out, "oalgpu_voice_readback", true)) return rc;
    const DeviceLayout &L = c->L;
    std::memset(out, 0, sizeof(*out));
    VoiceCtl ctl;
    HIP_TRY(hipMemcpy(&ctl, L.ctl + v, sizeof(ctl), hipMemcpyDeviceToHost));
    out->play_state = ctl.playState; out->position = ctl.position; out->position_frac = ctl.positionFrac;
    out->has_buffer = ctl.curBuffer >= 0; out->fading = (ctl.flags & kFlagFading) != 0;
    out->hrtf_old_gain = ctl.hrtfOldGain;
    out->hrtf_old_delay[0] = ctl.hrtfOldDelay[0]; out->hrtf_old_delay[1] = ctl.hrtfOldDelay[1];
    HIP_TRY(hipMemcpy(out->prev_samples, L.prev + size_t{v} * kMaxPad, sizeof(out->prev_samples), hipMemcpyDeviceToHost));
    HIP_TRY(hipMemcpy(out->hrtf_history, L.hist + size_t{v} * kHist, sizeof(out->hrtf_history), hipMemcpyDeviceToHost));
    if(!L.hrtf)
        HIP_TRY(hipMemcpy(out->dry_current, L.gainCur + size_t{v} * L.numDry, L.numDry * sizeof(float), hipMemcpyDeviceToHost));
    BiquadSlot slots[2 * OALGPU_MAX_SENDS];
    HIP_TRY(hipMemcpy(slots, L.dfilt + size_t{v} * 2, 2 * sizeof(BiquadSlot), hipMemcpyDeviceToHost));
    std::memcpy(&out->direct_lp, &slots[0].f, sizeof(oalgpu_biquad));
    std::memcpy(&out->direct_hp, &slots[1].f, sizeof(oalgpu_biquad));
    for(uint32_t s = 0; s < OALGPU_MAX_SENDS; ++s) { oalgpu_biquad_reset(&out->send_lp[s]); oalgpu_biquad_reset(&out->send_hp[s]); }
    if(L.numSends)
    {
        HIP_TRY(hipMemcpy(slots, L.sfilt + size_t{v} * L.numSends * 2, L.numSends * 2 * sizeof(BiquadSlot), hipMemcpyDeviceToHost));
        std::vector<float> cur(size_t{L.numSends} * L.wetChannels);
        HIP_TRY(hipMemcpy(cur.data(), L.sendCur + size_t{v} * L.numSends * L.wetChannels, cur.size() * sizeof(float), hipMemcpyDeviceToHost));
        for(uint32_t s = 0; s < L.numSends; ++s)
        {
            std::memcpy(&out->send_lp[s], &slots[s * 2].f, sizeof(oalgpu_biquad));
            std::memcpy(&out->send_hp[s], &slots[s * 2 + 1].f, sizeof(oalgpu_biquad));
            std::memcpy(out->send_current[s], cur.data() + size_t{s} * L.wetChannels, L.wetChannels * sizeof(float));
        }
    }
    return OALGPU_OK;
}

int oalgpu_voices_readback(oalgpu_context *c, const uint32_t *voices, size_t count, oalgpu_voice_brief *out)
{
    if(!c || !voices || !out) return Fail(OALGPU_ERR_INVALID, "oalgpu_voices_readback: null argument");
    if(count == 0) return OALGPU_OK;
    if(int rc = BeginVoiceCall(c, true, "", true)) return rc;
    uint32_t lo = 0xffffffffu, hi = 0u;
    for(size_t i = 0; i < count; ++i)
    {
        if(voices[i] >= c->L.numVoices) return Fail(OALGPU_ERR_INVALID, "oalgpu_voices_readback: bad voice index");
        lo = std::min(lo, voices[i]); hi = std::max(hi, voices[i]);
    }
    c->ctlHost.resize(size_t{hi - lo} + 1u);
    HIP_TRY(hipMemcpy(c->ctlHost.data(), c->L.ctl + lo, c->ctlHost.size() * sizeof(VoiceCtl), hipMemcpyDeviceToHost));
    for(size_t i = 0; i < count; ++i)
    {
        const VoiceCtl &ctl = c->ctlHost[voices[i] - lo];
        out[i] = oalgpu_voice_brief{ctl.playState, ctl.position, ctl.positionFrac, ctl.curBuffer >= 0 ? 1 : 0,
            (ctl.flags & kFlagFading) ? 1 : 0, ctl.curBuffer, 0u};
    }
    bool anyQueue = false;
    for(size_t i = 0; i < count; ++i) anyQueue = anyQueue || (c->ctlHost[voices[i] - lo].flags & kFlagQueue);
    if(anyQueue)
    {
        c->doneHost.resize(size_t{hi - lo} + 1u);
        HIP_TRY(hipMemcpy(c->doneHost.data(), c->queueDone.p + lo, c->doneHost.size() * sizeof(uint32_t), hipMemcpyDeviceToHost));
        for(size_t i = 0; i < count; ++i)
        {
            out[i].buffers_done = c->doneHost[voices[i] - lo];
            c->buf.noteQueueDone(voices[i], out[i].buffers_done);
        }
    }
    return OALGPU_OK;
}
```

openal-soft_amd/csrc/api_poststage.hip:

```cpp
#include "api_context.hpp"

static const char *const kPostNames[6] = {"nothing", "B-Format decoder", "front stabilizer", "crossfeed", "UHJ encoder", "TSME encoder"};

constexpr uint32_t Bit(PostKind k) { return 1u << uint32_t(k); }

static const uint32_t kAcceptedOver[6] = {
     Bit(PostKind::None) | Bit(PostKind::AmbiDec) | Bit(PostKind::Uhj) | Bit(PostKind::Tsme),
     Bit(PostKind::None) | Bit(PostKind::AmbiDec) | Bit(PostKind::Stabilizer) | Bit(PostKind::Bs2b),
     Bit(PostKind::AmbiDec) | Bit(PostKind::Stabilizer),
     Bit(PostKind::AmbiDec) | Bit(PostKind::Bs2b),
     Bit(PostKind::None) | Bit(PostKind::Uhj),
     Bit(PostKind::None) | Bit(PostKind::Tsme),
};

static const char kAttachedHasNoPostStage[] = "the context is attached (oalgpu_context_attach): its device context has the post stage";

static int CheckPost(const oalgpu_context *c, const char *who, PostKind want)
{
    const std::string w = std::string(who) + ": ";
    if(c->L.hrtf) return Fail(OALGPU_ERR_INVALID, w + "an HRTF context post-processes with MixDirectHrtf");
    if(c->attachedTo && want != PostKind::None) return Fail(OALGPU_ERR_INVALID, w + kAttachedHasNoPostStage);
    if(kAcceptedOver[uint32_t(want)] & Bit(c->post)) return OALGPU_OK;
    const char *have = kPostNames[uint32_t(c->post)];
    if(want == PostKind::None) return Fail(OALGPU_ERR_INVALID, w + "the context's " + have + " decodes with it (remove that first)");
    if(c->post == PostKind::None) return Fail(OALGPU_ERR_INVALID, w + "needs a B-Format decoder (oalgpu_set_bformat_decoder)");
    return Fail(OALGPU_ERR_INVALID, w + "the context post-processes with its " + have);
}

static void RemovePost(oalgpu_context *c, PostKind kind)
{
    if(c->post != kind) return;
    c->post = (kind == PostKind::Stabilizer || kind == PostKind::Bs2b) ? PostKind::AmbiDec : PostKind::None;
}

int oalgpu_set_bformat_decoder(oalgpu_context *c, uint32_t num_out, const float *coeffs_hf, const float *coeffs_lf,
    float xover_norm)
{
    static const char who[] = "oalgpu_set_bformat_decoder";
    if(!c) return Fail(OALGPU_ERR_INVALID, "null argument");
    if(c->L.hrtf) return Fail(OALGPU_ERR_INVALID, "oalgpu_set_bformat_decoder: an HRTF context post-processes with MixDirectHrtf");
    if(int rc = UseCtx(c)) return rc;
    if(int rc = oalgpu_sync(c)) return rc;
    const bool on = num_out != 0 && coeffs_hf;
    if(int rc = CheckPost(c, who, on ? PostKind::AmbiDec : PostKind::None)) return rc;
    if(!on) { RemovePost(c, PostKind::AmbiDec); return OALGPU_OK; }
    if(num_out > c->L.numReal || num_out > 32u)
        return Fail(OALGPU_ERR_INVALID, "oalgpu_set_bformat_decoder: more output channels than real output lines");
    if(coeffs_lf && !(xover_norm > 0.0f && xover_norm < 0.5f))
        return Fail(OALGPU_ERR_INVALID, "oalgpu_set_bformat_decoder: a dual-band decoder needs 0 < xover_norm < 0.5");
    const uint32_t nin = c->L.numDry;
    std::vector<float> hf(size_t{nin} * 32, 0.0f), lf(size_t{nin} * 32, 0.0f);
    for(uint32_t j = 0; j < nin && j < OALGPU_MAX_AMBI_CHANNELS; ++j)
        for(uint32_t o = 0; o < num_out; ++o)
        {
            hf[j * 32 + o] = coeffs_hf[size_t{o} * OALGPU_MAX_AMBI_CHANNELS + j];
            if(coeffs_lf) lf[j * 32 + o] = coeffs_lf[size_t{o} * OALGPU_MAX_AMBI_CHANNELS + j];
        }
    HIP_TRY(c->decGainsHf.alloc(hf.size())); HIP_TRY(c->decGainsHf.upload(hf.data(), hf.size()));
    HIP_TRY(c->decGainsLf.alloc(lf.size())); HIP_TRY(c->decGainsLf.upload(lf.data(), lf.size()));
    HIP_TRY(c->decBands.alloc(size_t{nin} * 2 * kLine)); HIP_TRY(c->decBands.zero());
    std::vector<SplitterState> sp(nin);
    for(auto &s : sp) s = SplitterState{coeffs_lf ? SplitterCoeff(xover_norm) : 0.0f, 0.0f, 0.0f, 0.0f};
    HIP_TRY(c->decSplit.alloc(nin)); HIP_TRY(c->decSplit.upload(sp.data(), nin));
    c->decOut = num_out; c->decDual = coeffs_lf != nullptr;
    if(c->post == PostKind::None) c->post = PostKind::AmbiDec;
    return OALGPU_OK;
}

int oalgpu_limiter_device_params(uint32_t sample_rate, int sample_type, float dither_depth, oalgpu_limiter_params *out)
{
    if(!out || sample_rate == 0 || sample_type < OALGPU_OUT_I8 || sample_type > OALGPU_OUT_F32 || !(dither_depth >= 0.0f))
        return Fail(OALGPU_ERR_INVALID, "oalgpu_limiter_device_params: bad arguments");
    return LimiterDeviceParams(sample_rate, sample_type, dither_depth, out) ? 1 : 0;
}

uint32_t oalgpu_limiter_look_ahead(const oalgpu_limiter_params *params)
{
    LimiterConsts k{};
    if(!params || !LimiterDerive(*params, &k)) return 0u;
    return k.lookAhead;
}

int oalgpu_set_output_limiter(oalgpu_context *c, const oalgpu_limiter_params *params)
{
    if(int rc = BeginSetter(c, "oalgpu_set_output_limiter")) return rc;
    if(params && c->attachedTo) return Fail(OALGPU_ERR_INVALID, std::string("oalgpu_set_output_limiter: ") + kAttachedHasNoPostStage);
    const uint32_t nlines = RealOutLines(c);
    LimiterConsts k{};
    if(params)
    {
        if(params->num_channels != 0 && params->num_channels != nlines)
            return Fail(OALGPU_ERR_INVALID, "oalgpu_set_output_limiter: num_channels is not the context's number of output lines");
        if(!LimiterDerive(*params, &k))
            return Fail(OALGPU_ERR_INVALID, "oalgpu_set_output_limiter: bad parameters");
        k.numChans = nlines;
    }
    if(int rc = oalgpu_sync(c)) return rc;
    c->limOn = false;
    if(params)
    {
        std::vector<float> init(LimiterStateFloats(nlines), 0.0f);
        std::fill(init.begin() + kLimiterHoldHistory, init.begin() + kLimiterHoldHistory + kLine, -INFINITY);
        HIP_TRY(c->limState.alloc(init.size()));
        HIP_TRY(c->limState.upload(init.data(), init.size()));
        c->lim = k;
        c->limOn = true;
    }
    if(c->outFloats) c->outRing = RingEligible(c);
    return OALGPU_OK;
}

int RunLimiter(oalgpu_context *c, hipStream_t s, uint32_t samplesToDo)
{
    if(!c->limOn) return OALGPU_OK;
    LaunchLimiter(s, RealOut(c), samplesToDo, c->lim, c->limState.p);
    HIP_TRY(hipGetLastError());
    return OALGPU_OK;
}

static int SetStereoEncoder(oalgpu_context *c, const char *who, PostKind kind, uint32_t needDry, int quality)
{
    if(int rc = BeginSetter(c, who)) return rc;
    if(quality >= 0)
    {
        if(UhjEncoderDelay(quality) == 0)
            return Fail(OALGPU_ERR_INVALID, std::string(who) + ": not a quality of the " + kPostNames[uint32_t(kind)]);
        if(int rc = CheckPost(c, who, kind)) return rc;
        if(c->L.numDry != needDry || c->L.numReal != 2)
            return Fail(OALGPU_ERR_INVALID, std::string(who) + ": needs " + (needDry == 3 ? "three dry lines (W, X, Y)" : "four dry lines (W, Y, Z, X)")
                + " and two real output lines");
    }
    if(int rc = oalgpu_sync(c)) return rc;
    RemovePost(c, kind);
    if(quality >= 0)
    {
        if(const uint32_t len = UhjFirLength(quality))
        {
            const std::vector<float> taps = UhjFirTaps(len);
            HIP_TRY(c->encTaps.alloc(taps.size()));
            HIP_TRY(c->encTaps.upload(taps.data(), taps.size()));
        }
        HIP_TRY(c->encState.alloc(UhjStateFloats(quality)));
        HIP_TRY(c->encState.zero());
        c->encQuality = quality;
        c->post = kind;
    }
    return OALGPU_OK;
}

uint32_t oalgpu_uhj_encoder_delay(int quality) { return UhjEncoderDelay(quality); }
uint32_t oalgpu_tsme_encoder_delay(int quality) { return UhjEncoderDelay(quality); }
int oalgpu_set_uhj_encoder(oalgpu_context *c, int quality) { return SetStereoEncoder(c, "oalgpu_set_uhj_encoder", PostKind::Uhj, 3, quality); }
int oalgpu_set_tsme_encoder(oalgpu_context *c, int quality) { return SetStereoEncoder(c, "oalgpu_set_tsme_encoder", PostKind::Tsme, 4, quality); }

int oalgpu_front_stabilizer_constants(float xover_norm, float *out)
{
    StabilizerConsts k{};
    if(!out || !StabilizerDerive(xover_norm, &k))
        return Fail(OALGPU_ERR_INVALID, "oalgpu_front_stabilizer_constants: needs 0 < xover_norm < 0.5");
    out[0] = k.coeff; out[1] = k.midLf; out[2] = k.midHf; out[3] = k.centerLf; out[4] = k.centerHf;
    return OALGPU_OK;
}

int oalgpu_set_front_stabilizer(oalgpu_context *c, const oalgpu_stabilizer_params *params)
{
    static const char who[] = "oalgpu_set_front_stabilizer";
    if(int rc = BeginSetter(c, who)) return rc;
    StabilizerConsts k{};
    if(params)
    {
        if(int rc = CheckPost(c, who, PostKind::Stabilizer)) return rc;
        const uint32_t nr = c->L.numReal;
        if(nr > 32u || params->left >= nr || params->right >= nr || params->center >= nr || params->left == params->right
            || params->left == params->center || params->right == params->center)
            return Fail(OALGPU_ERR_INVALID, "oalgpu_set_front_stabilizer: left, right and center are three different real output lines");
        if(!StabilizerDerive(params->xover_norm, &k))
            return Fail(OALGPU_ERR_INVALID, "oalgpu_set_front_stabilizer: needs 0 < xover_norm < 0.5");
    }
    if(int rc = oalgpu_sync(c)) return rc;
    RemovePost(c, PostKind::Stabilizer);
    if(params)
    {
        HIP_TRY(c->stabState.alloc(kStabilizerStateFloats));
        HIP_TRY(c->stabState.zero());
        c->stab = k;
        c->stabLeft = params->left; c->stabRight = params->right; c->stabCenter = params->center;
        c->post = PostKind::Stabilizer;
    }
    return OALGPU_OK;
// ... 119 lines not shown
```

openal-soft_amd/csrc/api_resident.hip:

```cpp
#include "api_context.hpp"

namespace {
std::mutex gResLock;
std::vector<oalgpu_context*> gResRunning;
std::atomic<int> gResCount{0};

void ResidentEnter(oalgpu_context *c)
{
    c->res.running = true;
    gResRunning.push_back(c);
    gResCount.store(int(gResRunning.size()), std::memory_order_relaxed);
}
void ResidentLeave(oalgpu_context *c)
{
    c->res.running = false;
    gResRunning.erase(std::remove(gResRunning.begin(), gResRunning.end(), c), gResRunning.end());
    gResCount.store(int(gResRunning.size()), std::memory_order_relaxed);
}

void ResidentParkLocked(oalgpu_context *c)
{
    auto &R = c->res;
    if(!R.running) return;
    __atomic_store_n(&R.door->exitSeq[R.launches & 3u], R.next, __ATOMIC_RELEASE);
// ... 142 lines not shown
        }
        else (void)hipGetLastError();
    }
    return ResidentGiveUp(c, std::string(e < 4 ? what[e] : "a wait timed out") + state);
}

int ResidentSubmit(oalgpu_context *c, uint32_t samples_to_do)
{
    auto &R = c->res;
    if(!R.ready) { if(int rc = ResidentInit(c)) return R.failed ? 1 : rc; }
    HIP_TRY(hipSetDevice(c->desc.device));
    std::unique_lock<std::mutex> g(gResLock);
    const DeviceLayout &L = c->L;
    const bool launchNow = !R.running;
    ResidentArgs a{};
    uint32_t evk = 0;
    bool timed = false;
    if(launchNow)
    {
        if(c->postPending) HIP_TRY(hipStreamWaitEvent(R.reduceStream, c->lastPostEvent ? c->lastPostEvent : c->evPostDone, 0));
        const uint32_t k = evk = R.launches % oalgpu_context::ResidentState::kEv;
        if(R.evOpen[k]) { HIP_TRY(hipEventSynchronize(R.evStop[k])); ResidentCollectTimes(c, false); }
        timed = R.timeLaunches;
        a.door = R.door; a.counters = R.counters.p; a.hostFlags = R.hostFlags; a.partBase = R.part.p; a.setStride = uint32_t(R.setFloats);
        a.base = R.next; a.endSeq = R.next + R.maxUpdates; a.redPerUpdate = R.redGroups;
        a.startedTarget = R.startedTotal + L.numGroups; a.launchId = R.launches + 1u;
        __atomic_store_n(&R.door->exitSeq[a.launchId & 3u], R.next + 0x40000000u, __ATOMIC_RELEASE);
        __atomic_store_n(&R.door->seq, R.next, __ATOMIC_RELEASE);
        __builtin_ia32_sfence();
    }
    if(!SpinFiveSeconds([&] { return int32_t(R.posts - __atomic_load_n(R.hostFlags + 16u * kRhProgress, __ATOMIC_ACQUIRE)) < int32_t(kResidentDepth); }))
    {
        ResidentParkLocked(c);
        g.unlock();
        ResidentDrain(c);
        if(int rc = ResidentCheckError(c)) return rc;
        return ResidentGiveUp(c, "the post-process made no progress for 5 s");
    }
    if(__atomic_load_n(R.hostFlags + 16u * kRhError, __ATOMIC_RELAXED))
    {
        ResidentParkLocked(c);
        g.unlock();
        ResidentDrain(c);
        return ResidentCheckError(c);
    }
    c->outRingWritten = false;
    oalgpu_param_block *b = R.pendingBlock;
    R.pendingBlock = nullptr;
    if(b) b->heldBy = nullptr;
    ResidentSlot &sl = R.door->slot[R.next % kResidentSlots];
    sl.recs = b ? reinterpret_cast<unsigned long long>(b->recs.p) : 0ull;
    sl.map = b ? reinterpret_cast<unsigned long long>(b->voiceToRec.p) : 0ull;
    sl.rows = b ? reinterpret_cast<unsigned long long>(b->rows.p) : 0ull;
    sl.samples = samples_to_do;
    __builtin_ia32_sfence();
    __atomic_store_n(&R.door->seq, R.next + 1u, __ATOMIC_RELEASE);
    __builtin_ia32_sfence();
    if(launchNow)
    {
        const uint32_t k = evk;
        HIP_TRY(LaunchVoiceWaveResident(c->stream, L, a, timed ? R.evStart[k] : nullptr, timed ? R.evStop[k] : nullptr));
        R.evOpen[k] = timed; R.evFirst[k] = R.next; R.evLast[k] = R.next;
        ++R.launches; R.startedTotal = a.startedTarget; R.endSeq = a.endSeq; R.launchBase = R.next;
        R.awaitStarted = a.launchId;
        ResidentEnter(c);
    }
    const uint32_t set = R.next % kResidentSets;
    if(R.awaitStarted)
    {
        const uint32_t id = R.awaitStarted;
        R.awaitStarted = 0u;
        if(!SpinFiveSeconds([&] { return __atomic_load_n(R.hostFlags + 16u * kRhResident, __ATOMIC_ACQUIRE) == id; }))
        {
            ++R.next;
            ResidentParkLocked(c);
            g.unlock();
            (void)hipStreamSynchronize(c->stream);
            return ResidentGiveUp(c, "its workgroups did not all start within 5 s");
        }
    }
    if(R.copyPending) { HIP_TRY(hipStreamWaitEvent(R.reduceStream, R.copyPending, 0)); R.copyPending = nullptr; }
    DeviceLayout Lr = L;
    Lr.partHrtf = R.part.p + size_t{set} * R.setFloats;
    LaunchBusReduceResident(R.reduceStream, Lr, CarrySource(c, true), R.counters.p, R.hostFlags, set, (R.setUses[set] + 1u) * L.numGroups,
        R.posts * R.firGroups);
    HIP_TRY(hipGetLastError());
    ++R.setUses[set];
    c->lastPostEvent = c->evPostDone;
    if(int rc = PostDirectHrtfFused(c, c->postStream, samples_to_do, c->limOn ? nullptr : c->evPostDone, true)) return rc;
    if(c->limOn)
    {
        if(int rc = RunLimiter(c, c->postStream, samples_to_do)) return rc;
        HIP_TRY(hipEventRecord(c->evPostDone, c->postStream));
        R.copyPending = c->evPostDone;
    }
    c->postPending = true;
    ++R.next;
    ++c->updatesSubmitted;
    R.evLast[(R.launches - 1u) % oalgpu_context::ResidentState::kEv] = R.next;
    if(R.next == R.endSeq) ResidentLeave(c);
    return OALGPU_OK;
}

int oalgpu_resident_stats(oalgpu_context *c, oalgpu_resident_info *out)
{
    if(!c || !out) return Fail(OALGPU_ERR_INVALID, "null argument");
    auto &R = c->res;
    uint32_t w[kRcCount * 16] = {};
    if(R.ready && !R.running)
    {
        if(int rc = UseDevice(c->desc.device)) return rc;
        HIP_TRY(hipMemcpy(w, R.counters.p, sizeof(w), hipMemcpyDeviceToHost));
    }
    std::lock_guard<std::mutex> g(gResLock);
    out->enabled = R.enabled ? 1 : 0; out->failed = R.failed ? 1 : 0; out->running = R.running ? 1 : 0;
    out->door_in_device_memory = R.doorInBar ? 1 : 0;
    out->launches = R.launches; out->updates = R.next; out->parks = uint32_t(R.parks);
    out->timed_launches = uint32_t(R.kernelLaunches); out->timed_updates = R.kernelUpdates; out->timed_kernel_ms = R.kernelMs;
    out->max_updates_per_launch = R.maxUpdates; out->pad = 0;
    const double tick = 0.01, groups = double(std::max<uint32_t>((c->L.numGroups + 127u) / 128u, 1u));
    out->wait_door_us = w[16 * kRcWaitDoor] * tick / groups; out->wait_reduction_us = w[16 * kRcWaitRed] * tick / groups;
    out->wait_arrival_us = w[16 * kRcWaitArrive] * tick; out->wait_post_us = w[16 * kRcWaitPost] * tick;
    out->wait_reduced_us = w[16 * kRcWaitRedDone] * tick; out->wait_split_us = w[16 * kRcWaitSplit] * tick;
    out->install_us = w[16 * kRcInstall] * tick / groups; out->busy_us = w[16 * kRcBusy] * tick / groups;
    out->top_us = w[16 * kRcTop] * tick / groups;
    return OALGPU_OK;
}

int oalgpu_resident_set_short_run(oalgpu_context *c, uint32_t updates)
{
    if(!c) return Fail(OALGPU_ERR_INVALID, "null argument");
    if(int rc = UseCtx(c)) return rc;
    c->res.shortRun = updates;
    c->res.shortRuns = 0; c->res.cooldown = 0;
    return OALGPU_OK;
}

int oalgpu_resident_set_timing(oalgpu_context *c, int enable)
{
    if(!c) return Fail(OALGPU_ERR_INVALID, "null argument");
    if(int rc = UseCtx(c)) return rc;
    c->res.timeLaunches = enable != 0;
    return OALGPU_OK;
}

int oalgpu_resident_set_max_updates(oalgpu_context *c, uint32_t max_updates)
{
    if(!c || max_updates == 0 || max_updates > 0x10000000u) return Fail(OALGPU_ERR_INVALID, "oalgpu_resident_set_max_updates: 1 .. 2^28");
    if(int rc = UseCtx(c)) return rc;
    c->res.maxUpdates = max_updates;
    return OALGPU_OK;
}
```

openal-soft_amd/csrc/dev_reduce.hpp:

```cpp
#pragma once
#include "kernels.hpp"

namespace oalgpu {

constexpr int kReduceSegs = 16;

template<bool COHERENT>
__device__ __forceinline__ void ReduceStore(float *p, float v)
{
    if constexpr (COHERENT) __hip_atomic_store(p, v, __ATOMIC_RELAXED, __HIP_MEMORY_SCOPE_AGENT);
    else *p = v;
}

template<bool COHLOAD, class P>
__device__ __forceinline__ float ReduceLoad(P p)
{
    if constexpr (COHLOAD) return __hip_atomic_load(p, __ATOMIC_RELAXED, __HIP_MEMORY_SCOPE_AGENT);
    else return *p;
}
struct ReduceNoHook { __device__ __forceinline__ void operator()() const { } };

template<int kReduceWaves, bool COHERENT, int KF = 8, bool COHLOAD = false, class MID = ReduceNoHook>
__device__ __forceinline__ void BusReduceBlock(const DeviceLayout &L, const float *__restrict__ carry, float (*slice)[64], uint32_t block, uint32_t tid,
    MID mid = MID{})
// ... 41 lines not shown
        uint32_t common = per;
#pragma unroll
        for(int q = 0; q < 4; ++q)
        {
            const uint32_t seg = wave0 + 4u * uint32_t(q);
            gA[q] = seg * per < ngroups ? seg * per : ngroups;
            gE[q] = (gA[q] + per < ngroups) ? gA[q] + per : ngroups;
            oo[q] = (off + gA[q] * stride) * 4u;
            sum[q] = 0.0f;
            common = (gE[q] - gA[q]) < common ? gE[q] - gA[q] : common;
        }
        if(have)
        {
#pragma unroll 1
            for(uint32_t j = 0; j + uint32_t(KF) <= common; j += uint32_t(KF))
            {
                float v[4][KF];
#pragma unroll
                for(int q = 0; q < 4; ++q)
#pragma unroll
                    for(int k = 0; k < KF; ++k) v[q][k] = ReduceLoad<COHLOAD>(reinterpret_cast<gfloatp>(reinterpret_cast<gcharp>(base) + (oo[q] + uint32_t(k) * sb)));
#pragma unroll
                for(int q = 0; q < 4; ++q)
                {
#pragma unroll
                    for(int k = 0; k < KF; ++k) sum[q] = sum[q] + v[q][k];
                    oo[q] += uint32_t(KF) * sb; gA[q] += uint32_t(KF);
                }
            }
#pragma unroll
            for(int q = 0; q < 4; ++q)
                for(; gA[q] < gE[q]; ++gA[q]) { sum[q] = sum[q] + ReduceLoad<COHLOAD>(reinterpret_cast<gfloatp>(reinterpret_cast<gcharp>(base) + oo[q])); oo[q] += sb; }
        }
        mid();
        float t = (carry && idx >= lineFloats && idx < total) ? ReduceLoad<COHLOAD>(carry + (idx - lineFloats)) : 0.0f;
#pragma unroll
        for(int q = 0; q < 4; ++q)
        {
            slice[wave0][lane] = sum[q];
            __syncthreads();
            if(wave0 == 0) { t = t + slice[0][lane]; t = t + slice[1][lane]; t = t + slice[2][lane]; t = t + slice[3][lane]; }
            __syncthreads();
        }
        if(wave0 == 0 && idx < total && (idx < lineFloats || L.hrtf)) ReduceStore<COHERENT>(&L.bus[idx], t);
        return;
    }
    else
#pragma unroll 1
    for(uint32_t seg = wave0; seg < uint32_t(kReduceSegs); seg += kReduceWaves)
    {
        const uint32_t g0 = seg * per < ngroups ? seg * per : ngroups;
        const uint32_t g1 = (g0 + per < ngroups) ? g0 + per : ngroups;
        float sum = 0.0f;
        if(have)
        {
            typedef const __attribute__((address_space(1))) char *gcharp;
            const uint32_t sb = stride * 4u;
            uint32_t g = g0, o = (off + g0 * stride) * 4u;
#pragma unroll 1
            for(; g + 8 <= g1; g += 8)
            {
                float v[8];
#pragma unroll
                for(int k = 0; k < 8; ++k) v[k] = *reinterpret_cast<gfloatp>(reinterpret_cast<gcharp>(base) + (o + uint32_t(k) * sb));
#pragma unroll
                for(int k = 0; k < 8; ++k) sum = sum + v[k];
                o += 8u * sb;
            }
            for(; g < g1; ++g) { sum = sum + *reinterpret_cast<gfloatp>(reinterpret_cast<gcharp>(base) + o); o += sb; }
        }
        slice[seg][lane] = sum;
    }
    __syncthreads();
    if(wave0 == 0 && idx < total)
    {
        float t = (carry && idx >= lineFloats) ? carry[idx - lineFloats] : 0.0f;
        t = t + slice[0][lane];
#pragma unroll 5
        for(int w = 1; w < kReduceSegs; ++w) t = t + slice[w][lane];
        if(idx < lineFloats || L.hrtf) ReduceStore<COHERENT>(&L.bus[idx], t);
    }
}

}
```

openal-soft_amd/csrc/kernels.hpp:

```cpp
#pragma once
#include <hip/hip_runtime.h>
#include <stdint.h>

#include "dev_hrtf.hpp"
#include "dev_mix.hpp"
#include "dev_resample.hpp"
#include "dev_voice.hpp"
#include "../host/limiter_params.hpp"
#include "../host/uhj_params.hpp"
#include "../host/stabilizer_params.hpp"
#include "../host/crossfeed_params.hpp"

namespace oalgpu {

enum VoiceFlagBits : uint32_t {
    kFlagFading = 1u << 0,
    kFlagHasHrtf = 1u << 1,
    kFlagDirectFilter = 1u << 2,
    kFlagHrtfDirty = 1u << 3,
    kFlagAmbiScale = 1u << 4,
    kFlagNfc = 1u << 5,
    kFlagQueue = 1u << 7,
    kFlagDelayed = 1u << 6,
    kFlagSendFilterShift = 8
// ... 137 lines not shown
        const uint32_t i = (lane - 8) >> 1, hp = (lane - 8) & 1u;
        BiquadSetTarget(L.sfilt[(size_t{v} * L.numSends + i) * 2 + hp].f, hp ? r.sendHp[i] : r.sendLp[i]);
    }
    if(L.hrtf) { if(!r.keepHrtf) ApplyHrtfTargetWave(L, v, r.hrtfIdx, r.hrtfW, r.hrtfPass, lane); }
    else if(lane < L.numDry)
        L.gainTgt[size_t{v} * L.numDry + lane] = r.dryGains[lane];
    for(uint32_t k = lane; k < L.numSends * L.wetChannels; k += 64)
        L.sendTgt[size_t{v} * L.numSends * L.wetChannels + k] = r.sendGains[k / L.wetChannels][k % L.wetChannels];
}

struct VoiceInitRecord { uint32_t voice; int32_t buffer, looping, position; uint32_t positionFrac; int32_t queue; };

constexpr uint32_t kResidentSets = 4;
constexpr uint32_t kResidentSlots = 16;
constexpr uint32_t kResidentDepth = 8;
constexpr unsigned long long kResidentWatchdogTicks = 200000000ull;

struct ResidentSlot { unsigned long long recs, map, rows; uint32_t samples, pad; };
struct alignas(64) ResidentDoor {
    uint32_t seq;
    uint32_t exitSeq[4];
    uint32_t pad[11];
    ResidentSlot slot[kResidentSlots];
};
enum ResidentCounter : uint32_t {
    kRcArrive0 = 0,
    kRcRedRead = 4,
    kRcRedDone = 5,
    kRcPostDone = 6,
    kRcStarted = 7,
    kRcWaitDoor = 8,
    kRcWaitRed = 9,
    kRcWaitArrive = 10,
    kRcWaitPost = 11,
    kRcWaitRedDone = 12,
    kRcWaitSplit = 13,
    kRcInstall = 14,
    kRcBusy = 15,
    kRcTop = 16,
    kRcCount = 17
};
enum ResidentHostFlag : uint32_t { kRhResident = 0, kRhError = 1, kRhProgress = 2,
    kRhFault = 3,
    kRhCount = 4 };
struct ResidentArgs {
    const ResidentDoor *door;
    uint32_t *counters;
    uint32_t *hostFlags;
    float *partBase;
    uint32_t setStride;
    uint32_t base, endSeq;
    uint32_t redPerUpdate;
    uint32_t startedTarget, launchId;
};

void LaunchResample(hipStream_t s, bool exact, const ResampleSpec &spec, const float *src, uint32_t frac,
    uint32_t increment, float *dst, uint32_t n);
void LaunchMix(hipStream_t s, const float *in, uint32_t n, float *out, uint32_t nlines, float *cur,
    const float *tgt, uint32_t counter, uint32_t outpos);
void LaunchMixHrtf(hipStream_t s, bool exact, const float *in, float *accum, uint32_t irsize, const float *coeffs,
    uint32_t dL, uint32_t dR, float gain, float step, const float *oldcoeffs, uint32_t odL, uint32_t odR,
    float oldgain, int blend, uint32_t n);
void LaunchMixDirectHrtf(hipStream_t s, bool exact, float *left, float *right, const float *in, uint32_t nch,
    float *accum, SplitterState *splitters, const float *hfscales, const float *chanCoeffs, uint32_t irsize,
    uint32_t n, float *temp);
void LaunchBiquadDual(hipStream_t s, BiquadState *f0, BiquadState *f1, const float *src, float *dst, uint32_t n);
void LaunchGetCoeffs(hipStream_t s, const HrtfStoreDev &st, const float *dirs, uint32_t count, float *coeffs,
    uint32_t *delays);

void LaunchPostDirectHrtfFast(hipStream_t s, float *left, float *right, const float *in, uint32_t nch, float *accum,
    SplitterState *splitters, const float *hfscales, const float *chanCoeffs, uint32_t irsize, uint32_t n, float *temp,
    hipEvent_t evDone = nullptr);

inline uint32_t ReducePostReduceGroups(const DeviceLayout &L) { return uint32_t((BusFloats(L) + 63u) / 64u); }
struct PostHrtfCall {
    float *left, *right; const float *in; uint32_t nch; const float *accIn; float *carryOut;
    const SplitterState *spIn; SplitterState *spOut; const float *hfscales, *chanCoeffs; uint32_t irsize, n;
    float *xf; uint32_t *arrived; uint32_t epoch; const float *runPower; hipEvent_t evDone;
    float *hostOut; uint32_t *hostFlag; uint32_t hostSeq;
};
void LaunchReducePostFused(hipStream_t s, const PostHrtfCall &p, const DeviceLayout &L, const float *carry, uint32_t *outArrived, uint32_t outTarget,
    uint32_t *reduced, uint32_t reducedEpoch);
void LaunchPostDirectHrtfFused(hipStream_t s, const PostHrtfCall &p, uint32_t *outArrived, uint32_t outTarget);
void LaunchBusReduceResident(hipStream_t s, const DeviceLayout &L, const float *carry, uint32_t *counters, uint32_t *hostFlags, uint32_t set,
    uint32_t arriveTarget, uint32_t postDoneTarget);
uint32_t PostResidentFirGroups();
void LaunchPostResident(hipStream_t s, const PostHrtfCall &p, uint32_t *counters, uint32_t *hostFlags, uint32_t redDoneTarget, uint32_t postDoneTarget,
    uint32_t progressValue);

void LaunchBFormatDecode(hipStream_t s, bool exact, float *out, const float *lines, SplitterState *states, float *bands,
    const float *gainsHf, const float *gainsLf, uint32_t nin, uint32_t nout, uint32_t n);
void LaunchDither(hipStream_t s, float *lines, uint32_t nlines, uint32_t n, float quantScale, uint32_t seed);
uint32_t DitherAdvanceSeed(uint32_t seed, uint32_t draws);
void LaunchWriteSamples(hipStream_t s, int sampleType, const float *lines, uint32_t nlines, uint32_t n, uint32_t frameStep, void *out);
void LaunchLimiter(hipStream_t s, float *lines, uint32_t n, const LimiterConsts &k, float *state);
size_t LimiterStateFloats(uint32_t nch);
constexpr size_t kLimiterHoldHistory = 16u + 1024u;
void LaunchUhjEncode(hipStream_t s, int quality, float *left, float *right, const float *w, const float *x, const float *y,
    uint32_t n, const float *taps, float *state);
size_t UhjStateFloats(int quality);
void LaunchTsmeEncode(hipStream_t s, int quality, float *left, float *right, const float *dry, uint32_t n, const float *taps,
    float *state);
constexpr size_t kStabilizerScratch = 64;
constexpr size_t kStabilizerStateFloats = kStabilizerScratch + 2 * kLine;
void LaunchStabilizerSplit(hipStream_t s, float *real, uint32_t lidx, uint32_t ridx, uint32_t n, float *state);
void LaunchStabilizer(hipStream_t s, float *real, uint32_t numReal, uint32_t lidx, uint32_t ridx, uint32_t cidx, uint32_t n,
    const StabilizerConsts &k, float *state);
void LaunchDistanceComp(hipStream_t s, float *lines, uint32_t nlines, uint32_t n, const uint32_t *delays, const float *gains,
    float *hist);
constexpr size_t kCrossfeedScratch = 64;
constexpr size_t kCrossfeedStateFloats = kCrossfeedScratch + 2 * kLine;
void LaunchCrossfeedSplit(hipStream_t s, float *real, uint32_t lidx, uint32_t ridx, uint32_t n, float *state);
void LaunchCrossfeed(hipStream_t s, float *real, uint32_t lidx, uint32_t ridx, uint32_t n, const CrossfeedConsts &k, float *state);
constexpr uint32_t kFxMaxIn = 16;
struct FxState {
    BiquadState bq[kFxMaxIn][4];
    float cur[64];
    float env;
};
struct FxLaunch {
    int kind, exact;
    uint32_t numIn, nlines, n;
    FxState *st;
    const float *wetIn; float *outLines;
    uint32_t target[kFxMaxIn]; float tgtGain[kFxMaxIn];
    const float *tgtGains;
    uint32_t modIndex, modRange; float modScale; int modWave;
    float *delay; uint32_t delayMask, offset, tap[2]; float feedGain;
    int compOn; float attackMult, releaseMult;
};
void LaunchEffect(hipStream_t s, const FxLaunch &F);

struct Fx2State {
    float cur[kFxMaxIn];
    float upCur[9][32];
    float split[9][3];
    BiquadState lp[4], bp[4];
    float envDelay, awZ[kFxMaxIn][2];
    float vmS[kFxMaxIn][8][2];
};
struct FsPair { double x, y; };
struct Fx2Launch {
    int kind;
    uint32_t numIn, nlines, n;
    Fx2State *st;
    const float *wetIn; float *outLines;
    uint32_t target[kFxMaxIn]; float tgtGain[kFxMaxIn];
    int upsample; float hfScale[2], splitCoeff; const float *upTgt;
    int chWave; uint32_t lfoStart[2], lfoRange; float lfoScale, chDepth; int32_t chDelay; float chFeedback;
    uint32_t chAvgDelay, chHist;
    float *delay; uint32_t delayMask, offset; const float *cubic;
    float edgeCoeff;
    float attackRate, releaseRate, resonanceGain, peakGain, freqMinNorm, bandwidthNorm;
    int vmWave; uint32_t vmIndex, vmStep; float vmG[8], vmGain[8];
    double *fsIn; FsPair *fsOutFifo, *fsAccum, *fsOutdata; const FsPair *fsTw, *fsPhase; const float *fsWindow;
    uint32_t fsCount, fsPos, fsPhaseStep[4], fsPhaseIdx[4]; double fsSign[4];
    const float *psRingIn; float *psRingOut;
    const float *psPhaseIn; float *psPhaseOut;
    float *psAccum, *psOutFifo, *psRows;
    const float *psTw, *psWindow;
    uint32_t psCount, psPos, psPitchI; float psPitch;
};
void LaunchEffect2(hipStream_t s, const Fx2Launch &F, uint32_t ldsBytes);

struct ConvertChunk { uint32_t srcBase, frac0, dstBase, dstSize; };
struct ConvertJob {
// ... 78 lines not shown
```

openal-soft_amd/csrc/post_wave.hip:

```cpp
#include <hip/hip_ext.h>
#include "dev_wave.hpp"
#include "dev_reduce.hpp"

#pragma clang fp contract(off)

namespace oalgpu {
namespace {

constexpr int kPostFrames = kLine + kHrirLen;
constexpr int kPostGroup = 4;

__global__ void OALGPU_SINGLE_DS_OPS __launch_bounds__(64) __attribute__((amdgpu_num_vgpr(32))) PostSplitKernel(const float *__restrict__ in, float *__restrict__ xf,
    SplitterState *__restrict__ splitters, const float *__restrict__ hfscales, uint32_t n)
{
    __shared__ float x[kLine + 64];
    const uint32_t c = blockIdx.x, lane = threadIdx.x;
    for(uint32_t k = lane; k < uint32_t(kLine); k += 64) x[k] = (k < n) ? in[size_t{c} * kLine + k] : 0.0f;
    WaveSync();
    SplitterState st = splitters[c];
    SplitterScanHfTri(st, x, n, hfscales[c], lane);
    if(lane == 0) splitters[c] = st;
    WaveSync();
    for(uint32_t k = lane; k < uint32_t(kLine); k += 64) xf[size_t{c} * kLine + k] = (k < n) ? x[k] : 0.0f;
}
// ... 258 lines not shown
                __hip_atomic_store(hostFlag, hostSeq, __ATOMIC_RELEASE, __HIP_MEMORY_SCOPE_SYSTEM);
            }
        }
    }
}

__global__ void OALGPU_SINGLE_DS_OPS __launch_bounds__(64) __attribute__((amdgpu_num_vgpr(48))) PostFusedKernel(const float *__restrict__ in, uint32_t nch,
    const SplitterState *__restrict__ spIn, SplitterState *__restrict__ spOut, const float *__restrict__ hfscales,
    const float *__restrict__ chanCoeffs, uint32_t taps, const float *__restrict__ accIn, float *__restrict__ carryOut,
    float *__restrict__ left, float *__restrict__ right, uint32_t n, float *__restrict__ xf, uint32_t *__restrict__ arrived, uint32_t epoch,
    Tri3 runPower, float *__restrict__ hostOut, uint32_t *__restrict__ hostFlag, uint32_t hostSeq, uint32_t *__restrict__ outArrived, uint32_t outTarget)
{
    __shared__ float xs[kLine + 64];
    __builtin_amdgcn_s_setprio(3);
    PostFusedBlock<0>(xs, blockIdx.x, threadIdx.x, outTarget, in, nch, spIn, spOut, hfscales, chanCoeffs, taps, accIn, carryOut, left, right, n,
        xf, arrived, epoch, runPower, hostOut, hostFlag, hostSeq, outArrived, nullptr, 0u);
}

#ifndef OALGPU_FUSED_KF
#define OALGPU_FUSED_KF 4
#endif
struct ReducePostArgs {
    const float *carry; uint32_t nReduce;
    const float *in; uint32_t nch;
    const SplitterState *spIn; SplitterState *spOut; const float *hfscales, *chanCoeffs; uint32_t taps;
    const float *accIn; float *carryOut, *left, *right; uint32_t n; float *xf; uint32_t *arrived; uint32_t epoch; Tri3 runPower;
    float *hostOut; uint32_t *hostFlag; uint32_t hostSeq; uint32_t *outArrived; uint32_t outTarget;
    uint32_t *reduced; uint32_t reducedEpoch;
};
__global__ void OALGPU_SINGLE_DS_OPS __launch_bounds__(256) __attribute__((amdgpu_num_vgpr(48))) ReducePostFusedKernel(DeviceLayout L, ReducePostArgs A)
{
    __shared__ float xs[kLine + 64];
    if(blockIdx.x < A.nReduce)
    {
        BusReduceBlock<4, true, OALGPU_FUSED_KF>(L, A.carry, reinterpret_cast<float (*)[64]>(xs), blockIdx.x, threadIdx.x);
        if(threadIdx.x < 64)
        {
            asm volatile("s_waitcnt vmcnt(0)" ::: "memory");
            if(threadIdx.x == 0) __hip_atomic_fetch_add(A.reduced, 1u, __ATOMIC_RELAXED, __HIP_MEMORY_SCOPE_AGENT);
        }
        return;
    }
    if(threadIdx.x >= 64) return;
    PostFusedBlock<1>(xs, blockIdx.x - A.nReduce, threadIdx.x, A.outTarget, A.in, A.nch, A.spIn, A.spOut, A.hfscales, A.chanCoeffs, A.taps,
        A.accIn, A.carryOut, A.left, A.right, A.n, A.xf, A.arrived, A.epoch, A.runPower, A.hostOut, A.hostFlag, A.hostSeq, A.outArrived, A.reduced, A.reducedEpoch);
}

struct ResidentReduceArgs {
    uint32_t *counters, *hostFlags;
    uint32_t set, arriveTarget, postDoneTarget;
};
__global__ void __launch_bounds__(256) __attribute__((amdgpu_num_vgpr(48))) BusReduceResidentKernel(DeviceLayout L, const float *__restrict__ carry,
    ResidentReduceArgs A)
{
    __shared__ float slice[4][64];
    const uint32_t tid = threadIdx.x;
    __builtin_amdgcn_s_setprio(3);
    if(tid == 0)
    {
        if(!PostWaitCounter(A.counters + 16u * (kRcArrive0 + A.set), A.arriveTarget, 4, blockIdx.x == 0 ? A.counters + 16u * kRcWaitArrive : nullptr))
            __hip_atomic_store(A.hostFlags + 16u * kRhError, 2u, __ATOMIC_RELAXED, __HIP_MEMORY_SCOPE_SYSTEM);
    }
    __syncthreads();
    auto mid = [&]()
    {
        asm volatile("s_waitcnt vmcnt(0)" ::: "memory");
        __syncthreads();
        if(tid == 0)
        {
            __hip_atomic_fetch_add(A.counters + 16u * kRcRedRead, 1u, __ATOMIC_RELAXED, __HIP_MEMORY_SCOPE_AGENT);
            if(!PostWaitCounter(A.counters + 16u * kRcPostDone, A.postDoneTarget, 4, blockIdx.x == 0 ? A.counters + 16u * kRcWaitPost : nullptr))
                __hip_atomic_store(A.hostFlags + 16u * kRhError, 3u, __ATOMIC_RELAXED, __HIP_MEMORY_SCOPE_SYSTEM);
        }
        __syncthreads();
    };
    BusReduceBlock<4, true, 8, true>(L, carry, slice, blockIdx.x, tid, mid);
    if(tid < 64)
    {
        asm volatile("s_waitcnt vmcnt(0)" ::: "memory");
        if(tid == 0) __hip_atomic_fetch_add(A.counters + 16u * kRcRedDone, 1u, __ATOMIC_RELAXED, __HIP_MEMORY_SCOPE_AGENT);
    }
}

__global__ void OALGPU_SINGLE_DS_OPS __launch_bounds__(64) __attribute__((amdgpu_num_vgpr(48))) PostResidentKernel(const float *__restrict__ in, uint32_t nch,
    const SplitterState *__restrict__ spIn, SplitterState *__restrict__ spOut, const float *__restrict__ hfscales,
    const float *__restrict__ chanCoeffs, uint32_t taps, const float *__restrict__ accIn, float *__restrict__ carryOut,
    float *__restrict__ left, float *__restrict__ right, uint32_t n, float *__restrict__ xf, uint32_t *__restrict__ arrived, uint32_t epoch,
    Tri3 runPower, float *__restrict__ hostOut, uint32_t *__restrict__ hostFlag, uint32_t hostSeq, const uint32_t *__restrict__ reduced,
    uint32_t reducedEpoch, PostResident PR)
{
    __shared__ float xs[kLine + 64];
    __builtin_amdgcn_s_setprio(3);
    PostFusedBlock<2>(xs, blockIdx.x, threadIdx.x, 0u, in, nch, spIn, spOut, hfscales, chanCoeffs, taps, accIn, carryOut, left, right, n,
        xf, arrived, epoch, runPower, hostOut, hostFlag, hostSeq, nullptr, reduced, reducedEpoch, PR);
}

}

void LaunchBusReduceResident(hipStream_t s, const DeviceLayout &L, const float *carry, uint32_t *counters, uint32_t *hostFlags, uint32_t set,
    uint32_t arriveTarget, uint32_t postDoneTarget)
{
    const uint32_t total = uint32_t(BusFloats(L));
    hipLaunchKernelGGL(BusReduceResidentKernel, dim3((total + 63u) / 64u), dim3(256), 0, s, L, carry, ResidentReduceArgs{counters, hostFlags, set, arriveTarget, postDoneTarget});
}

static uint32_t PostTaps(uint32_t irsize) { return irsize <= 16u ? 16u : ((irsize + 15u) & ~15u); }
static Tri3 PostRunPower(const PostHrtfCall &p) { return Tri3{p.runPower[0], p.runPower[1], p.runPower[2], p.runPower[3]}; }

uint32_t PostResidentFirGroups() { return uint32_t(kPostFrames / kFusedFrames); }
void LaunchPostResident(hipStream_t s, const PostHrtfCall &p, uint32_t *counters, uint32_t *hostFlags, uint32_t redDoneTarget, uint32_t postDoneTarget,
    uint32_t progressValue)
{
    const PostResident PR{counters + 16u * kRcPostDone, postDoneTarget, hostFlags + 16u * kRhProgress, progressValue, hostFlags + 16u * kRhError, counters};
    hipExtLaunchKernelGGL(PostResidentKernel, dim3(p.nch + kPostFrames / kFusedFrames), dim3(64), 0, s, nullptr, p.evDone, 0u, p.in, p.nch, p.spIn, p.spOut,
        p.hfscales, p.chanCoeffs, PostTaps(p.irsize), p.accIn, p.carryOut, p.left, p.right, p.n, p.xf, p.arrived, p.epoch, PostRunPower(p), p.hostOut,
        p.hostFlag, p.hostSeq, counters + 16u * kRcRedDone, redDoneTarget, PR);
}

void LaunchPostDirectHrtfFused(hipStream_t s, const PostHrtfCall &p, uint32_t *outArrived, uint32_t outTarget)
{
    static_assert(kPostFrames % kFusedFrames == 0, "whole workgroups");
    hipExtLaunchKernelGGL(PostFusedKernel, dim3(p.nch + kPostFrames / kFusedFrames), dim3(64), 0, s, nullptr, p.evDone, 0u, p.in, p.nch, p.spIn, p.spOut,
        p.hfscales, p.chanCoeffs, PostTaps(p.irsize), p.accIn, p.carryOut, p.left, p.right, p.n, p.xf, p.arrived, p.epoch, PostRunPower(p), p.hostOut,
        p.hostFlag, p.hostSeq, outArrived, outTarget);
}

void LaunchReducePostFused(hipStream_t s, const PostHrtfCall &p, const DeviceLayout &L, const float *carry, uint32_t *outArrived, uint32_t outTarget,
    uint32_t *reduced, uint32_t reducedEpoch)
{
    ReducePostArgs A{};
    A.carry = carry; A.nReduce = ReducePostReduceGroups(L);
    A.in = p.in; A.nch = p.nch; A.spIn = p.spIn; A.spOut = p.spOut; A.hfscales = p.hfscales; A.chanCoeffs = p.chanCoeffs;
    A.taps = PostTaps(p.irsize);
    A.accIn = p.accIn; A.carryOut = p.carryOut; A.left = p.left; A.right = p.right; A.n = p.n; A.xf = p.xf; A.arrived = p.arrived; A.epoch = p.epoch;
    A.runPower = PostRunPower(p);
    A.hostOut = p.hostOut; A.hostFlag = p.hostFlag; A.hostSeq = p.hostSeq; A.outArrived = outArrived; A.outTarget = outTarget; A.reduced = reduced; A.reducedEpoch = reducedEpoch;
    hipExtLaunchKernelGGL(ReducePostFusedKernel, dim3(A.nReduce + p.nch + kPostFrames / kFusedFrames), dim3(256), 0, s, nullptr, p.evDone, 0u, L, A);
}

void LaunchPostDirectHrtfFast(hipStream_t s, float *left, float *right, const float *in, uint32_t nch, float *accum,
    SplitterState *splitters, const float *hfscales, const float *chanCoeffs, uint32_t irsize, uint32_t n, float *temp, hipEvent_t evDone)
{
    float *xf = temp, *tmp = temp + size_t{nch} * kLine;
    const uint32_t taps = PostTaps(irsize);
    hipLaunchKernelGGL(PostSplitKernel, dim3(nch), dim3(64), 0, s, in, xf, splitters, hfscales, n);
    hipLaunchKernelGGL(PostFirKernel<16>, dim3(kPostFrames / 16), dim3(64), 0, s, xf, nch, chanCoeffs, taps, tmp);
    hipExtLaunchKernelGGL(PostShiftKernel, dim3(1), dim3(256), 0, s, nullptr, evDone, 0u, left, right, accum, tmp, n);
}

}
```

openal-soft_amd/oalgpu/__init__.py:

```python
import ctypes as C
import os

import numpy as np

PKG_DIR = os.path.dirname(os.path.dirname(os.path.abspath(__file__)))
LIB_PATH = os.path.join(PKG_DIR, "liboalgpu.so")

BUFFER_LINE = 1024
MAX_PAD = 48
HRTF_HIST = 64
HRIR_LEN = 128
MAX_SENDS = 6
(OUT_I8, OUT_U8, OUT_I16, OUT_U16, OUT_I32, OUT_U32, OUT_F32) = range(7)
MAX_OUT = 32
MAX_AMBI = 25
MATH_EXACT, MATH_FAST = 0, 1
(RS_POINT, RS_LINEAR, RS_SPLINE, RS_GAUSSIAN, RS_FAST_BSINC12, RS_BSINC12, RS_FAST_BSINC24,
 RS_BSINC24, RS_FAST_BSINC48, RS_BSINC48) = range(10)
FMT_UBYTE, FMT_SHORT, FMT_INT, FMT_FLOAT, FMT_DOUBLE, FMT_MULAW, FMT_ALAW = range(7)
FMT_DTYPES = {FMT_UBYTE: np.uint8, FMT_SHORT: np.int16, FMT_INT: np.int32, FMT_FLOAT: np.float32,
              FMT_DOUBLE: np.float64, FMT_MULAW: np.uint8, FMT_ALAW: np.uint8}
VOICE_STOPPED, VOICE_PLAYING, VOICE_STOPPING, VOICE_PENDING = range(4)

f32p = C.POINTER(C.c_float)
MOVE_DTYPE = np.dtype([("voice", np.uint32), ("hrtf_ev", np.float32), ("hrtf_az", np.float32), ("hrtf_dist", np.float32),
                       ("hrtf_spread", np.float32), ("hrtf_gain", np.float32)])
u32p = C.POINTER(C.c_uint32)


class OalgpuError(RuntimeError):
    pass


class BsincTable(C.Structure):
    _fields_ = [("scaleBase", C.c_float), ("scaleRange", C.c_float), ("m", C.c_uint32 * 16),
                ("filterOffset", C.c_uint32 * 16), ("tab", f32p), ("tablen", C.c_size_t)]


class InterpState(C.Structure):
    _fields_ = [("kind", C.c_int32), ("table", C.c_int32), ("sf", C.c_float), ("m", C.c_uint32),
                ("l", C.c_uint32), ("filter_offset", C.c_uint32)]


class Biquad(C.Structure):
    _fields_ = [(n, C.c_float) for n in ("z1", "z2", "b0", "b1", "b2", "a1", "a2", "tb0", "tb1",
                                         "tb2", "ta1", "ta2")] + [("counter", C.c_int32)]

    def as_tuple(self):
        return tuple(getattr(self, n) for n, _ in self._fields_)


class Splitter(C.Structure):
    _fields_ = [("coeff", C.c_float), ("lp_z1", C.c_float), ("lp_z2", C.c_float),
                ("ap_z1", C.c_float)]


class HrtfInfo(C.Structure):
    _fields_ = [(n, C.c_uint32) for n in ("sample_rate", "ir_size", "num_fields", "num_elevs",
                                          "num_irs")]


class ContextDesc(C.Structure):
    _fields_ = [("device", C.c_int32), ("math_mode", C.c_int32), ("sample_rate", C.c_uint32),
                ("num_dry_channels", C.c_uint32), ("num_real_channels", C.c_uint32),
                ("num_aux_sends", C.c_uint32), ("num_slots", C.c_uint32),
                ("wet_channels", C.c_uint32), ("hrtf", C.c_int32), ("max_voices", C.c_uint32),
                ("max_buffers", C.c_uint32), ("voices_per_group", C.c_uint32), ("flags", C.c_uint32)]


class VoiceEvent(C.Structure):
    _fields_ = [("voice", C.c_uint32), ("play_state", C.c_int32), ("has_buffer", C.c_int32), ("current_buffer", C.c_int32),
                ("buffers_done", C.c_uint32), ("position", C.c_int32), ("position_frac", C.c_uint32), ("fading", C.c_int32)]


CTX_FIR_VALU, CTX_PROFILE, CTX_SERIAL, CTX_STREAM_ROWS, CTX_APPLY_IN_VOICE_KERNEL, CTX_FUSED_REDUCE = 1, 2, 4, 8, 16, 32
CTX_RESIDENT = 64
CTX_SLICE_LINES = 128
CTX_WAVE_PAIRS = 256
CTX_ROW_SLICES = 512


class VoiceDesc(C.Structure):
    _fields_ = [("buffer", C.c_int32), ("looping", C.c_int32), ("position", C.c_int32),
                ("position_frac", C.c_uint32), ("frequency", C.c_uint32)]


class FilterParams(C.Structure):
    _fields_ = [("active", C.c_int32), ("gain_hf", C.c_float), ("hf_norm", C.c_float),
                ("gain_lf", C.c_float), ("lf_norm", C.c_float)]


class VoiceParams(C.Structure):
    _fields_ = [("step", C.c_uint32), ("resampler", C.c_int32), ("direct_filter", FilterParams),
                ("dry_gains", C.c_float * MAX_OUT),
                ("hrtf_ev", C.c_float), ("hrtf_az", C.c_float), ("hrtf_dist", C.c_float),
                ("hrtf_spread", C.c_float), ("hrtf_gain", C.c_float),
                ("send_slot", C.c_int32 * MAX_SENDS), ("send_filter", FilterParams * MAX_SENDS),
                ("send_gains", (C.c_float * MAX_AMBI) * MAX_SENDS)]


(DISTANCE_DISABLE, DISTANCE_INVERSE, DISTANCE_INVERSE_CLAMPED, DISTANCE_LINEAR, DISTANCE_LINEAR_CLAMPED, DISTANCE_EXPONENT,
 DISTANCE_EXPONENT_CLAMPED) = range(7)


class ListenerParams(C.Structure):
    _fields_ = [("matrix", C.c_float * 16), ("position", C.c_float * 3), ("velocity", C.c_float * 3),
                ("gain", C.c_float), ("meters_per_unit", C.c_float), ("air_absorption_gain_hf", C.c_float),
                ("doppler_factor", C.c_float), ("speed_of_sound", C.c_float),
                ("source_distance_model", C.c_int32), ("distance_model", C.c_int32),
                ("cone_scale", C.c_float), ("nfc_scale", C.c_float), ("xyz_scale", C.c_float * 3)]

    @classmethod
    def default(cls):
        p = cls()
        p.matrix[:] = [1, 0, 0, 0, 0, 1, 0, 0, 0, 0, 1, 0, 0, 0, 0, 1]
        p.gain, p.meters_per_unit, p.air_absorption_gain_hf, p.doppler_factor, p.speed_of_sound = 1.0, 1.0, 0.99426, 1.0, 343.3
        p.source_distance_model, p.distance_model = 0, DISTANCE_DISABLE
        p.cone_scale, p.nfc_scale = 1.0, 1.0
        p.xyz_scale[:] = [1.0, 1.0, 1.0]
        return p


class SlotEnvironment(C.Structure):
    _fields_ = [("active", C.c_int32), ("room_rolloff", C.c_float), ("decay_time", C.c_float), ("air_absorption_gain_hf", C.c_float)]


class SourceSend(C.Structure):
    _fields_ = [("slot", C.c_int32), ("gain", C.c_float), ("gain_hf", C.c_float), ("hf_reference", C.c_float),
                ("gain_lf", C.c_float), ("lf_reference", C.c_float)]


class SourceProps(C.Structure):
    _fields_ = [(n, C.c_float) for n in ("pitch", "gain", "outer_gain", "min_gain", "max_gain", "inner_angle", "outer_angle",
                                         "ref_distance", "max_distance", "rolloff_factor")] + [
        ("position", C.c_float * 3), ("velocity", C.c_float * 3), ("direction", C.c_float * 3),
        ("head_relative", C.c_int32), ("distance_model", C.c_int32), ("resampler", C.c_int32),
        ("dry_gain_hf_auto", C.c_int32), ("wet_gain_auto", C.c_int32), ("wet_gain_hf_auto", C.c_int32)] + [
        (n, C.c_float) for n in ("outer_gain_hf", "air_absorption_factor", "room_rolloff_factor", "doppler_factor", "radius",
                                 "direct_gain", "direct_gain_hf", "direct_hf_reference", "direct_gain_lf", "direct_lf_reference")] + [
        ("send", SourceSend * MAX_SENDS)]


def _params_host(name, per_source, desc, listener, sources, frequency, slots, dry_map, wet_maps, mhr):
    n = len(sources)
    out = (VoiceParams * (n * per_source))()
    u8p = C.POINTER(C.c_uint8)
    fn = getattr(lib, name)
    fn.argtypes = [C.POINTER(ContextDesc), C.POINTER(ListenerParams), C.c_void_p, u8p, f32p, u8p, f32p,
                   C.c_char_p, C.c_size_t, C.c_uint32, C.c_void_p, C.c_size_t, C.c_void_p]

    def maps(m):
        if m is None:
            return None, None, None
        idx = np.ascontiguousarray(m[0], np.uint8); sc = np.ascontiguousarray(m[1], np.float32)
        return idx.ctypes.data_as(u8p), _fp(sc), (idx, sc)
    di, ds, keep_d = maps(dry_map)
    wi, ws, keep_w = maps(wet_maps)
    check(fn(C.byref(desc), C.byref(listener), C.cast(slots, C.c_void_p) if slots is not None else None,
             di, ds, wi, ws, mhr, len(mhr) if mhr else 0, frequency, C.cast(sources, C.c_void_p), n, C.cast(out, C.c_void_p)), name)
    return out


# ... 719 lines not shown
        return out

    def set_slot_convolution(self, slot, conv):
        lib.oalgpu_slot_set_convolution.argtypes = [C.c_void_p, C.c_uint32, C.c_void_p]
        check(lib.oalgpu_slot_set_convolution(self.h, slot, conv.h if conv is not None else None))

    def set_slot_effect(self, slot, fx):
        lib.oalgpu_slot_set_effect.argtypes = [C.c_void_p, C.c_uint32, C.c_void_p]
        check(lib.oalgpu_slot_set_effect(self.h, slot, fx.h if fx is not None else None), "oalgpu_slot_set_effect")

    def set_slot_reverb(self, slot, rev):
        lib.oalgpu_slot_set_reverb.argtypes = [C.c_void_p, C.c_uint32, C.c_void_p]
        check(lib.oalgpu_slot_set_reverb(self.h, slot, rev.h if rev is not None else None))

    def set_slot_target(self, slot, target):
        lib.oalgpu_slot_set_target.argtypes = [C.c_void_p, C.c_uint32, C.c_int32]
        check(lib.oalgpu_slot_set_target(self.h, slot, -1 if target is None else target), "oalgpu_slot_set_target")

    def slot_target(self, slot):
        lib.oalgpu_slot_target.argtypes = [C.c_void_p, C.c_uint32, C.POINTER(C.c_int32)]
        t = C.c_int32(0)
        check(lib.oalgpu_slot_target(self.h, slot, C.byref(t)), "oalgpu_slot_target")
        return t.value

    def mix(self, samples_to_do=BUFFER_LINE, post_process=False):
        check(lib.oalgpu_mix_update(self.h, samples_to_do, 1 if post_process else 0),
              "oalgpu_mix_update")

    def sync(self):
        check(lib.oalgpu_sync(self.h), "oalgpu_sync")

    def resident_stats(self):
        class Info(C.Structure):
            _fields_ = [("enabled", C.c_int32), ("failed", C.c_int32), ("running", C.c_int32), ("door_in_device_memory", C.c_int32),
                        ("launches", C.c_uint32), ("updates", C.c_uint32), ("parks", C.c_uint32), ("timed_launches", C.c_uint32),
                        ("timed_updates", C.c_uint64), ("timed_kernel_ms", C.c_double),
                        ("max_updates_per_launch", C.c_uint32), ("pad", C.c_uint32),
                        ("wait_door_us", C.c_double), ("wait_reduction_us", C.c_double), ("wait_arrival_us", C.c_double),
                        ("wait_post_us", C.c_double), ("wait_reduced_us", C.c_double), ("wait_split_us", C.c_double),
                        ("install_us", C.c_double), ("busy_us", C.c_double), ("top_us", C.c_double)]
        info = Info()
        lib.oalgpu_resident_stats.argtypes = [C.c_void_p, C.POINTER(Info)]
        check(lib.oalgpu_resident_stats(self.h, C.byref(info)), "oalgpu_resident_stats")
        return {k: getattr(info, k) for k, _ in Info._fields_ if k != "pad"}

    def resident_set_short_run(self, updates):
        lib.oalgpu_resident_set_short_run.argtypes = [C.c_void_p, C.c_uint32]
        check(lib.oalgpu_resident_set_short_run(self.h, updates), "oalgpu_resident_set_short_run")

    def resident_set_timing(self, on):
        lib.oalgpu_resident_set_timing.argtypes = [C.c_void_p, C.c_int]
        check(lib.oalgpu_resident_set_timing(self.h, 1 if on else 0), "oalgpu_resident_set_timing")

    def resident_set_max_updates(self, n):
        lib.oalgpu_resident_set_max_updates.argtypes = [C.c_void_p, C.c_uint32]
        check(lib.oalgpu_resident_set_max_updates(self.h, n), "oalgpu_resident_set_max_updates")

    def dry(self):
        n = self.desc.num_dry_channels + self.desc.num_real_channels
        out = np.zeros((n, BUFFER_LINE), np.float32)
        check(lib.oalgpu_read_dry(self.h, _fp(out)), "oalgpu_read_dry")
        return out

    def wet(self, slot):
        out = np.zeros((self.desc.wet_channels, BUFFER_LINE), np.float32)
        check(lib.oalgpu_read_wet(self.h, slot, _fp(out)), "oalgpu_read_wet")
        return out

    def hrtf_accum(self):
        out = np.zeros((BUFFER_LINE + HRIR_LEN, 2), np.float32)
        check(lib.oalgpu_read_hrtf_accum(self.h, _fp(out)), "oalgpu_read_hrtf_accum")
        return out

    def voice_state(self, voice):
        st = VoiceState()
        check(lib.oalgpu_voice_readback(self.h, voice, C.byref(st)), "oalgpu_voice_readback")
        return st

    def bus_device_ptr(self):
        p, n, s = C.c_void_p(), C.c_size_t(), C.c_void_p()
        check(lib.oalgpu_bus_device_ptr(self.h, C.byref(p), C.byref(n), C.byref(s)))
        return p.value, n.value, s.value

    def voice_kernel_name(self):
        lib.oalgpu_voice_kernel_name.restype = C.c_char_p
        lib.oalgpu_voice_kernel_name.argtypes = [C.c_void_p]
        return lib.oalgpu_voice_kernel_name(self.h).decode()

    def set_timing(self, enable=True):
        check(lib.oalgpu_set_timing(self.h, 1 if enable else 0))

    def last_update_ms(self):
        a, b = C.c_float(), C.c_float()
        check(lib.oalgpu_last_update_ms(self.h, C.byref(a), C.byref(b)), "oalgpu_last_update_ms")
        return a.value, b.value


def comm_unique_id():
    buf = C.create_string_buffer(128)
    lib.oalgpu_comm_unique_id.argtypes = [C.c_char_p, C.c_size_t]
    check(lib.oalgpu_comm_unique_id(buf, 128), "oalgpu_comm_unique_id")
    return buf.raw


class Convolution:

    def __init__(self, num_out_lines, ir, device=0, ir_rate=None, device_rate=48000):
        lib.oalgpu_convolution_create_ex.argtypes = [C.c_int, C.c_uint32, f32p, C.c_uint32, C.c_uint32, C.c_uint32,
                                                     C.c_uint32, C.POINTER(C.c_void_p)]
        lib.oalgpu_convolution_set_channel_gains.argtypes = [C.c_void_p, f32p]
        lib.oalgpu_convolution_set_upsample.argtypes = [C.c_void_p, f32p, f32p, C.c_float]
        lib.oalgpu_convolution_destroy.argtypes = [C.c_void_p]
        lib.oalgpu_convolution_destroy.restype = None
        lib.oalgpu_convolution_set_target_gains.argtypes = [C.c_void_p, f32p]
        lib.oalgpu_convolution_process.argtypes = [C.c_void_p, f32p, f32p, C.c_uint32]
        lib.oalgpu_slot_set_convolution.argtypes = [C.c_void_p, C.c_uint32, C.c_void_p]
        self.nlines = num_out_lines
        ir = np.ascontiguousarray(ir, np.float32)
        self.channels = 1 if ir.ndim == 1 else ir.shape[1]
        h = C.c_void_p()
        check(lib.oalgpu_convolution_create_ex(device, num_out_lines, _fp(ir), ir.shape[0], self.channels,
                                               0 if ir_rate is None else ir_rate, 0 if ir_rate is None else device_rate,
                                               C.byref(h)), "oalgpu_convolution_create_ex")
        self.h = h

    def set_channel_gains(self, gains):
        g = np.ascontiguousarray(gains, np.float32).reshape(self.channels, -1)[:, :self.nlines]
        check(lib.oalgpu_convolution_set_channel_gains(self.h, _fp(np.ascontiguousarray(g))), "oalgpu_convolution_set_channel_gains")

    def set_upsample(self, hf_scales, lf_scales, xover_norm):
        if hf_scales is None:
            check(lib.oalgpu_convolution_set_upsample(self.h, None, None, 0.0))
            return
        hf = np.ascontiguousarray(hf_scales, np.float32)
        lf = np.ascontiguousarray(lf_scales, np.float32)
        check(lib.oalgpu_convolution_set_upsample(self.h, _fp(hf), _fp(lf), xover_norm), "oalgpu_convolution_set_upsample")

    def set_target_gains(self, gains):
        g = np.zeros(MAX_OUT, np.float32)
        g[:len(gains)] = gains
        check(lib.oalgpu_convolution_set_target_gains(self.h, _fp(g)))

    def process(self, wet_in, out_lines):
        wet_in = np.ascontiguousarray(wet_in, np.float32)
        assert out_lines.dtype == np.float32 and out_lines.shape == (self.nlines, BUFFER_LINE)
        check(lib.oalgpu_convolution_process(self.h, _fp(wet_in), _fp(out_lines), wet_in.size),
              "oalgpu_convolution_process")

    def close(self):
        if self.h:
            lib.oalgpu_convolution_destroy(self.h)
            self.h = None


(EFFECT_EQUALIZER, EFFECT_MODULATOR, EFFECT_ECHO, EFFECT_DEDICATED, EFFECT_COMPRESSOR, EFFECT_CHORUS, EFFECT_DISTORTION,
 EFFECT_AUTOWAH, EFFECT_VMORPHER, EFFECT_FSHIFTER, EFFECT_PSHIFTER) = range(11)
_EFFECT_INT_FIELDS = {EFFECT_MODULATOR: (2,), EFFECT_COMPRESSOR: (0,), EFFECT_CHORUS: (0, 1), EFFECT_VMORPHER: (1, 2, 3, 4, 5),
                      EFFECT_FSHIFTER: (1, 2), EFFECT_PSHIFTER: (0, 1)}
INVALID_CHANNEL = 0xffffffff


class Effect:

    def __init__(self, kind, num_out_lines, num_in=4, sample_rate=48000, mode=MATH_FAST, device=0):
        lib.oalgpu_effect_create.argtypes = [C.c_int, C.c_int, C.c_int, C.c_uint32, C.c_uint32, C.c_uint32, C.POINTER(C.c_void_p)]
        lib.oalgpu_effect_destroy.argtypes = [C.c_void_p]
# ... 161 lines not shown
```

Baseline: 108.9 million.

## Add short reduce-and-shift post path when dry bus is provably silent

Adds a ReduceShift kernel that, when the dry bus is known to carry nothing (HRTF only, no sends, slots, attachments, comm, limiter, dither or external bus access), reduces the per-group HRTF partials, writes the stereo output and shifts the HRTF carry in one launch. This replaces the full post stage, which runs the band splitter and direct-HRTF FIR over the dry channels. The carry is now double-buffered so the kernel can read one buffer while writing the other, and resident-mode counters are tracked as running totals. A dryLive flag, set by any API that could make the dry bus non-silent, guards the path. The risk is wrong output if some route that writes to the dry bus does not set the flag.

```diff
diff --git a/include/oalgpu.h b/include/oalgpu.h
--- a/include/oalgpu.h
+++ b/include/oalgpu.h
@@ -130,6 +130,7 @@
 #define OALGPU_CTX_WAVE_PAIRS 256u
 #define OALGPU_CTX_ROW_SLICES 512u
 #define OALGPU_CTX_SERIAL   4u
+#define OALGPU_CTX_FULL_POST 1024u
 
 int  oalgpu_context_create(const oalgpu_context_desc *desc, oalgpu_context **out);
 void oalgpu_context_destroy(oalgpu_context *ctx);
@@ -478,6 +479,11 @@
 
 const char *oalgpu_voice_kernel_name(oalgpu_context *ctx);
 
+#define OALGPU_POST_NONE  0
+#define OALGPU_POST_FULL  1
+#define OALGPU_POST_SHORT 2
+int oalgpu_last_post_path(oalgpu_context *ctx, int *path);
+
 typedef struct oalgpu_convolution oalgpu_convolution;
 int  oalgpu_convolution_create(int device, uint32_t num_out_lines, const float *ir, uint32_t ir_len,
     oalgpu_convolution **out);
diff --git a/openal-soft_amd/csrc/api.hip b/openal-soft_amd/csrc/api.hip
--- a/openal-soft_amd/csrc/api.hip
+++ b/openal-soft_amd/csrc/api.hip
@@ -249,6 +249,7 @@
     HIP_TRY(c->dSplit.alloc(L.numDry)); HIP_TRY(c->dSplit.zero());
     HIP_TRY(c->dSplit2.alloc(L.numDry)); HIP_TRY(c->dSplit2.zero());
     HIP_TRY(c->carryBuf.alloc(size_t{kLine + kHrirLen} * 2)); HIP_TRY(c->carryBuf.zero());
+    HIP_TRY(c->carryBuf2.alloc(size_t{kLine + kHrirLen} * 2)); HIP_TRY(c->carryBuf2.zero());
     HIP_TRY(c->postArrived.alloc(1)); HIP_TRY(c->postArrived.zero());
     HIP_TRY(c->dHfScale.alloc(L.numDry)); HIP_TRY(c->dHfScale.zero());
     HIP_TRY(c->dCoeffs.alloc(size_t{L.numDry} * kHrirLen * 2)); HIP_TRY(c->dCoeffs.zero());
@@ -291,7 +292,7 @@
 const float *CarrySource(oalgpu_context *c, bool carry)
 {
     const float *src = nullptr;
-    if(carry && c->L.hrtf) src = c->carryInBuf ? c->carryBuf.p : c->L.bus + BusAccumOffset(c->L);
+    if(carry && c->L.hrtf) src = c->carryInBuf ? c->carryBufAt(c->carryCur) : c->L.bus + BusAccumOffset(c->L);
     c->carryInBuf = false;
     return src;
 }
@@ -333,9 +334,9 @@
     if(resident)
     {
         c->reduceHeld = false;
-        LaunchPostResident(s, call, R.counters.p, R.hostFlags, (R.posts + 1u) * R.redGroups, (R.posts + 1u) * R.firGroups, R.posts + 1u);
+        LaunchPostResident(s, call, R.counters.p, R.hostFlags, R.redDoneTotal + R.redGroups, R.postDoneTotal + R.firGroups, R.posts + 1u);
         HIP_TRY(hipGetLastError());
-        ++R.posts;
+        ++R.posts; R.redDoneTotal += R.redGroups; R.postDoneTotal += R.firGroups;
     }
     else if(c->reduceHeld)
     {
@@ -357,7 +358,57 @@
     if(ring) c->outSlotSeq[slot] = ++c->outSeq;
     c->outRingWritten = ring;
     c->dSplitCur ^= 1u;
-    c->carryInBuf = true;
+    c->carryInBuf = true; c->carryCur = 0u;
+    c->lastPostPath = OALGPU_POST_FULL;
+    return OALGPU_OK;
+}
+
+bool SilentDry(const oalgpu_context *c)
+{
+    const DeviceLayout &L = c->L;
+    return !c->dryLive && !(c->desc.flags & OALGPU_CTX_FULL_POST) && L.hrtf && L.numSlots == 0 && L.numSends == 0 && L.accLines == 0 && !L.streams && !L.rows8
+        && L.numReal >= 2 && !c->comm && c->carryAccum && c->attached.empty() && !c->attachedTo && !c->timing && c->useWave && !c->exact;
+}
+
+int ReduceShift(oalgpu_context *c, hipStream_t s, const DeviceLayout &Lu, uint32_t samples_to_do, hipEvent_t evDone, bool resident)
+{
+    const DeviceLayout &L = c->L;
+    float *left = L.bus + size_t{L.numDry} * kLine;
+    const uint32_t slot = c->outNext % oalgpu_context::kIoSlots;
+    const bool ring = c->outRing && c->outFlags;
+    const uint32_t outTarget = c->outArrivedTotal + ReduceShiftOutGroups();
+    const float *src = CarrySource(c, true);
+    const uint32_t into = (src == c->carryBuf.p) ? 1u : 0u;
+    const ReduceShiftCall call{src, c->carryBufAt(into), left, left + kLine, samples_to_do, ring ? c->outHost[slot] : nullptr,
+        ring ? c->outFlags + size_t{slot} * 16 : nullptr, c->outSeq + 1u, c->outArrived.p, outTarget};
+    c->reduceHeld = false; c->shortHeld = false;
+    auto &R = c->res;
+    if(resident)
+    {
+        const uint32_t set = R.next % kResidentSets;
+        LaunchReduceShiftResident(s, Lu, call, R.counters.p, R.hostFlags, set, (R.setUses[set] + 1u) * L.numGroups, R.postDoneTotal, R.redGroups,
+            R.postDoneTotal + ReduceShiftGroups(), R.posts + 1u, evDone);
+        HIP_TRY(hipGetLastError());
+        ++R.setUses[set]; ++R.posts; R.postDoneTotal += ReduceShiftGroups();
+    }
+    else
+    {
+        LaunchReduceShift(s, Lu, call, evDone);
+        HIP_TRY(hipGetLastError());
+        if(ring) c->outArrivedTotal = outTarget;
+    }
+    if(ring) c->outSlotSeq[slot] = ++c->outSeq;
+    c->outRingWritten = ring;
+    c->carryInBuf = true; c->carryCur = into;
+    c->lastPostPath = OALGPU_POST_SHORT;
+    return OALGPU_OK;
+}
+
+int oalgpu_last_post_path(oalgpu_context *c, int *path)
+{
+    if(!c || !path) return Fail(OALGPU_ERR_INVALID, "null argument");
+    if(int rc = FlushPendingMix(c)) return rc;
+    *path = c->lastPostPath;
     return OALGPU_OK;
 }
 
@@ -454,6 +505,7 @@
         LaunchPostDirectHrtfFast(c->stream, left, right, L.bus, L.numDry, L.bus + BusAccumOffset(L), spCur,
             c->dHfScale.p, c->dCoeffs.p, c->dIrSize, samples_to_do, c->dTemp.p);
     HIP_TRY(hipGetLastError());
+    c->lastPostPath = OALGPU_POST_FULL;
     if(int rc = RunLimiter(c, c->stream, samples_to_do)) return rc;
     return EndTimedUpdate(c, c->stream);
 }
@@ -506,11 +558,12 @@
         if(post_process && c->commRank == 0) return oalgpu_post_process(c, samples_to_do);
         return OALGPU_OK;
     }
-    c->fuseReduce = post_process && !c->comm && c->L.hrtf && c->L.numSlots == 0 && c->L.numReal >= 2 && !c->timing
-        && (c->desc.flags & OALGPU_CTX_FUSED_REDUCE) && c->attached.empty();
+    c->shortHeld = post_process && c->commRank == 0 && SilentDry(c);
+    c->fuseReduce = c->shortHeld || (post_process && !c->comm && c->L.hrtf && c->L.numSlots == 0 && c->L.numReal >= 2 && !c->timing
+        && (c->desc.flags & OALGPU_CTX_FUSED_REDUCE) && c->attached.empty());
     const int rcv = oalgpu_mix_voices_overlapped(c, samples_to_do);
     c->fuseReduce = false;
-    if(rcv) { c->reduceHeld = false; return rcv; }
+    if(rcv) { c->reduceHeld = false; c->shortHeld = false; return rcv; }
     return oalgpu_post_process_overlapped(c, samples_to_do, post_process && c->commRank == 0);
 }
 
@@ -576,7 +629,8 @@
     {
         hipEvent_t ev = c->reduceHeld ? c->evReduceDone[c->heldParity] : ((c->timing || c->limOn) ? nullptr : c->evPostDone);
         c->lastPostEvent = (ev && !c->limOn) ? ev : c->evPostDone;
-        if(int rc = PostDirectHrtfFused(c, c->postStream, samples_to_do, ev)) return rc;
+        if(c->reduceHeld && c->shortHeld) { if(int rc = ReduceShift(c, c->postStream, c->heldL, samples_to_do, ev)) return rc; }
+        else if(int rc = PostDirectHrtfFused(c, c->postStream, samples_to_do, ev)) return rc;
         postDoneBound = ev != nullptr && !c->limOn;
         if(int rc = RunLimiter(c, c->postStream, samples_to_do)) return rc;
     }
diff --git a/openal-soft_amd/csrc/api_attach.hip b/openal-soft_amd/csrc/api_attach.hip
--- a/openal-soft_amd/csrc/api_attach.hip
+++ b/openal-soft_amd/csrc/api_attach.hip
@@ -95,6 +95,7 @@
     a->attachMap.assign(line_map, line_map + srcLines);
     a->attachedTo = d;
     d->attached.push_back(a);
+    NoteDryLive(d);
     if(int rc = RebuildMergeTable(d))
     {
         Unlink(a);
diff --git a/openal-soft_amd/csrc/api_comm.hip b/openal-soft_amd/csrc/api_comm.hip
--- a/openal-soft_amd/csrc/api_comm.hip
+++ b/openal-soft_amd/csrc/api_comm.hip
@@ -202,6 +202,7 @@
     if(r != ncclSuccess) return FailRccl("ncclCommInitRank", r);
     c->comm = t.release(); c->commRank = rank; c->commWorld = world;
     c->carryAccum = rank == 0;
+    NoteDryLive(c);
     return OALGPU_OK;
 }
 
@@ -287,6 +288,7 @@
     }
     c->comm = t.release(); c->commRank = rank; c->commWorld = world;
     c->carryAccum = rank == 0;
+    NoteDryLive(c);
     return OALGPU_OK;
 }
 
diff --git a/openal-soft_amd/csrc/api_context.hpp b/openal-soft_amd/csrc/api_context.hpp
--- a/openal-soft_amd/csrc/api_context.hpp
+++ b/openal-soft_amd/csrc/api_context.hpp
@@ -215,6 +215,11 @@
     const int32_t *nextMap{nullptr};
     const float *nextRows{nullptr};
     bool carryInBuf{false};
+    DevBuf<float> carryBuf2;
+    uint32_t carryCur{0};
+    float *carryBufAt(uint32_t k) { return k ? carryBuf2.p : carryBuf.p; }
+    bool dryLive{false}, shortHeld{false};
+    int lastPostPath{0};
     DevBuf<float> dHfScale, dCoeffs, dTemp;
     uint32_t dIrSize{0};
     bool directSet{false};
@@ -269,6 +274,7 @@
         uint32_t maxUpdates{4096};
         uint32_t setUses[kResidentSets]{};
         uint32_t posts{0};
+        uint32_t redDoneTotal{0}, postDoneTotal{0};
         uint32_t firGroups{0}, redGroups{0}, groupsPerCu{0};
         oalgpu_param_block *pendingBlock{nullptr};
         hipEvent_t copyPending{nullptr};
@@ -335,6 +341,9 @@
 int MixVoicesSerial(oalgpu_context *c, uint32_t samples_to_do);
 const float *CarrySource(oalgpu_context *c, bool carry);
 int PostDirectHrtfFused(oalgpu_context *c, hipStream_t s, uint32_t samples_to_do, hipEvent_t evDone, bool resident = false);
+bool SilentDry(const oalgpu_context *c);
+int ReduceShift(oalgpu_context *c, hipStream_t s, const DeviceLayout &L, uint32_t samples_to_do, hipEvent_t evDone, bool resident = false);
+inline void NoteDryLive(oalgpu_context *c) { c->dryLive = true; }
 int RebalanceWaveGroups(oalgpu_context *c);
 namespace oalgpu { void ParkResidentContexts(int device); }
 bool ResidentWanted(const oalgpu_context *c, int post_process);
diff --git a/openal-soft_amd/csrc/api_output.hip b/openal-soft_amd/csrc/api_output.hip
--- a/openal-soft_amd/csrc/api_output.hip
+++ b/openal-soft_amd/csrc/api_output.hip
@@ -166,6 +166,7 @@
     if(c->attachedTo && (sample_type != OALGPU_OUT_F32 || dither_depth > 0.0f))
         return Fail(OALGPU_ERR_INVALID, "oalgpu_set_output: the context is attached (oalgpu_context_attach): its device context has the post stage");
     c->outType = sample_type; c->ditherDepth = dither_depth; c->ditherSeed = dither_seed;
+    if(dither_depth > 0.0f && c->L.numReal > 2) NoteDryLive(c);
     return OALGPU_OK;
 }
 
@@ -206,7 +207,7 @@
 {
     if(!c || !out) return Fail(OALGPU_ERR_INVALID, "null argument");
     if(int rc = oalgpu_sync(c)) return rc;
-    HIP_TRY(hipMemcpy(out, c->carryInBuf ? c->carryBuf.p : c->L.bus + BusAccumOffset(c->L), size_t{kLine + kHrirLen} * 2 * sizeof(float), hipMemcpyDeviceToHost));
+    HIP_TRY(hipMemcpy(out, c->carryInBuf ? c->carryBufAt(c->carryCur) : c->L.bus + BusAccumOffset(c->L), size_t{kLine + kHrirLen} * 2 * sizeof(float), hipMemcpyDeviceToHost));
     return OALGPU_OK;
 }
 
@@ -216,6 +217,7 @@
     if(!ptr || !nfloats) return Fail(OALGPU_ERR_INVALID, "null argument");
     *ptr = c->L.bus;
     *nfloats = BusFloats(c->L);
+    NoteDryLive(c);
     if(hip_stream)
         *hip_stream = (c->useWave && c->ownStream && !c->serialOnly && c->postStream) ? c->postStream : c->stream;
     return OALGPU_OK;
diff --git a/openal-soft_amd/csrc/api_poststage.hip b/openal-soft_amd/csrc/api_poststage.hip
--- a/openal-soft_amd/csrc/api_poststage.hip
+++ b/openal-soft_amd/csrc/api_poststage.hip
@@ -105,6 +105,7 @@
         HIP_TRY(c->limState.upload(init.data(), init.size()));
         c->lim = k;
         c->limOn = true;
+        if(c->L.numReal > 2) NoteDryLive(c);
     }
     if(c->outFloats) c->outRing = RingEligible(c);
     return OALGPU_OK;
diff --git a/openal-soft_amd/csrc/api_resident.hip b/openal-soft_amd/csrc/api_resident.hip
--- a/openal-soft_amd/csrc/api_resident.hip
+++ b/openal-soft_amd/csrc/api_resident.hip
@@ -248,17 +248,25 @@
     if(R.copyPending) { HIP_TRY(hipStreamWaitEvent(R.reduceStream, R.copyPending, 0)); R.copyPending = nullptr; }
     DeviceLayout Lr = L;
     Lr.partHrtf = R.part.p + size_t{set} * R.setFloats;
-    LaunchBusReduceResident(R.reduceStream, Lr, CarrySource(c, true), R.counters.p, R.hostFlags, set, (R.setUses[set] + 1u) * L.numGroups,
-        R.posts * R.firGroups);
-    HIP_TRY(hipGetLastError());
-    ++R.setUses[set];
     c->lastPostEvent = c->evPostDone;
-    if(int rc = PostDirectHrtfFused(c, c->postStream, samples_to_do, c->limOn ? nullptr : c->evPostDone, true)) return rc;
-    if(c->limOn)
-    {
-        if(int rc = RunLimiter(c, c->postStream, samples_to_do)) return rc;
-        HIP_TRY(hipEventRecord(c->evPostDone, c->postStream));
-        R.copyPending = c->evPostDone;
+    if(SilentDry(c) && !c->limOn)
+    {
+        if(int rc = ReduceShift(c, R.reduceStream, Lr, samples_to_do, c->evPostDone, true)) return rc;
+        HIP_TRY(hipStreamWaitEvent(c->postStream, c->evPostDone, 0));
+    }
+    else
+    {
+        LaunchBusReduceResident(R.reduceStream, Lr, CarrySource(c, true), R.counters.p, R.hostFlags, set, (R.setUses[set] + 1u) * L.numGroups,
+            R.postDoneTotal);
+        HIP_TRY(hipGetLastError());
+        ++R.setUses[set];
+        if(int rc = PostDirectHrtfFused(c, c->postStream, samples_to_do, c->limOn ? nullptr : c->evPostDone, true)) return rc;
+        if(c->limOn)
+        {
+            if(int rc = RunLimiter(c, c->postStream, samples_to_do)) return rc;
+            HIP_TRY(hipEventRecord(c->evPostDone, c->postStream));
+            R.copyPending = c->evPostDone;
+        }
     }
     c->postPending = true;
     ++R.next;
diff --git a/openal-soft_amd/csrc/dev_reduce.hpp b/openal-soft_amd/csrc/dev_reduce.hpp
--- a/openal-soft_amd/csrc/dev_reduce.hpp
+++ b/openal-soft_amd/csrc/dev_reduce.hpp
@@ -147,4 +147,62 @@
     }
 }
 
-}
+template<bool COHERENT, bool COHLOAD, class MID = ReduceNoHook>
+__device__ __forceinline__ float AccumReduceBlock(const DeviceLayout &L, const float *__restrict__ carry, float (*slice)[64], uint32_t block, uint32_t wave,
+    uint32_t lane, MID mid = MID{})
+{
+    typedef const __attribute__((address_space(1))) float *gfloatp;
+    typedef const __attribute__((address_space(1))) char *gcharp;
+    constexpr uint32_t kCols = uint32_t(kLine + kHrirLen) * 2u, sb = kCols * 4u;
+    const uint32_t col = block * 64u + lane, voff = col * 4u;
+    const uint32_t ngroups = L.numGroups;
+    const uint32_t per = (ngroups + kReduceSegs - 1) / kReduceSegs;
+    const gcharp base = reinterpret_cast<gcharp>((const __attribute__((address_space(1))) void*)L.partHrtf);
+    uint32_t so[4], left[4];
+    float sum[4];
+    uint32_t common = per;
+#pragma unroll
+    for(int q = 0; q < 4; ++q)
+    {
+        const uint32_t seg = wave + 4u * uint32_t(q);
+        const uint32_t gA = seg * per < ngroups ? seg * per : ngroups;
+        const uint32_t gE = (gA + per < ngroups) ? gA + per : ngroups;
+        so[q] = gA * sb;
+        left[q] = gE - gA;
+        sum[q] = 0.0f;
+        common = left[q] < common ? left[q] : common;
+    }
+#pragma unroll 1
+    for(uint32_t j = 0; j + 8u <= common; j += 8u)
+    {
+        float v[4][8];
+#pragma unroll
+        for(int q = 0; q < 4; ++q)
+#pragma unroll
+            for(int k = 0; k < 8; ++k) v[q][k] = ReduceLoad<COHLOAD>(reinterpret_cast<gfloatp>(base + ((so[q] + uint32_t(k) * sb) + voff)));
+#pragma unroll
+        for(int q = 0; q < 4; ++q)
+        {
+#pragma unroll
+            for(int k = 0; k < 8; ++k) sum[q] = sum[q] + v[q][k];
+            so[q] += 8u * sb; left[q] -= 8u;
+        }
+    }
+#pragma unroll
+    for(int q = 0; q < 4; ++q)
+        for(; left[q]; --left[q]) { sum[q] = sum[q] + ReduceLoad<COHLOAD>(reinterpret_cast<gfloatp>(base + (so[q] + voff))); so[q] += sb; }
+    mid();
+    float t = carry ? ReduceLoad<COHLOAD>(carry + col) : 0.0f;
+#pragma unroll
+    for(int q = 0; q < 4; ++q)
+    {
+        slice[wave][lane] = sum[q];
+        __syncthreads();
+        if(wave == 0) { t = t + slice[0][lane]; t = t + slice[1][lane]; t = t + slice[2][lane]; t = t + slice[3][lane]; }
+        __syncthreads();
+    }
+    if(wave == 0) ReduceStore<COHERENT>(&L.bus[BusAccumOffset(L) + col], t);
+    return wave == 0 ? t : 0.0f;
+}
+
+}
diff --git a/openal-soft_amd/csrc/kernels.hpp b/openal-soft_amd/csrc/kernels.hpp
--- a/openal-soft_amd/csrc/kernels.hpp
+++ b/openal-soft_amd/csrc/kernels.hpp
@@ -243,6 +243,15 @@
 void LaunchReducePostFused(hipStream_t s, const PostHrtfCall &p, const DeviceLayout &L, const float *carry, uint32_t *outArrived, uint32_t outTarget,
     uint32_t *reduced, uint32_t reducedEpoch);
 void LaunchPostDirectHrtfFused(hipStream_t s, const PostHrtfCall &p, uint32_t *outArrived, uint32_t outTarget);
+struct ReduceShiftCall {
+    const float *carry; float *carryOut, *left, *right; uint32_t n;
+    float *hostOut; uint32_t *hostFlag; uint32_t hostSeq; uint32_t *outArrived; uint32_t outTarget;
+};
+uint32_t ReduceShiftGroups();
+uint32_t ReduceShiftOutGroups();
+void LaunchReduceShift(hipStream_t s, const DeviceLayout &L, const ReduceShiftCall &p, hipEvent_t evDone);
+void LaunchReduceShiftResident(hipStream_t s, const DeviceLayout &L, const ReduceShiftCall &p, uint32_t *counters, uint32_t *hostFlags, uint32_t set,
+    uint32_t arriveTarget, uint32_t postDoneBefore, uint32_t redGroups, uint32_t postDoneTarget, uint32_t progressValue, hipEvent_t evDone);
 void LaunchBusReduceResident(hipStream_t s, const DeviceLayout &L, const float *carry, uint32_t *counters, uint32_t *hostFlags, uint32_t set,
     uint32_t arriveTarget, uint32_t postDoneTarget);
 uint32_t PostResidentFirGroups();
diff --git a/openal-soft_amd/csrc/post_wave.hip b/openal-soft_amd/csrc/post_wave.hip
--- a/openal-soft_amd/csrc/post_wave.hip
+++ b/openal-soft_amd/csrc/post_wave.hip
@@ -364,6 +364,90 @@
     }
 }
 
+template<bool RESID>
+__device__ __forceinline__ void ReduceShiftColumn(const ReduceShiftCall &A, uint32_t col, float t)
+{
+    const uint32_t o = col >> 1, e = col & 1u, n = A.n;
+    auto put = [&](float *p, float v) { if constexpr (RESID) PostStoreCoherent(p, v); else *p = v; };
+    const float s = t + 0.0f;
+    if(o < uint32_t(kLine))
+    {
+        const float l = (o < n) ? 0.0f + s : 0.0f;
+        put((e ? A.right : A.left) + o, l);
+        if(A.hostOut) A.hostOut[e * uint32_t(kLine) + o] = l;
+    }
+    if(o >= n && o < n + uint32_t(kHrirLen)) put(A.carryOut + 2u * (o - n) + e, s);
+    if(o >= uint32_t(kHrirLen)) put(A.carryOut + 2u * o + e, (o < uint32_t(kHrirLen) + n) ? 0.0f : s);
+}
+constexpr uint32_t kShiftGroups = uint32_t(kPostFrames) * 2u / 64u;
+constexpr uint32_t kShiftOutGroups = uint32_t(kLine) * 2u / 64u;
+
+__global__ void __launch_bounds__(256) __attribute__((amdgpu_num_vgpr(48))) ReduceShiftKernel(DeviceLayout L, ReduceShiftCall A)
+{
+    __shared__ float slice[4][64];
+    __builtin_amdgcn_s_setprio(3);
+    const float t = AccumReduceBlock<false, false>(L, A.carry, slice, blockIdx.x, __builtin_amdgcn_readfirstlane(threadIdx.x >> 6), threadIdx.x & 63u);
+    if(threadIdx.x >= 64) return;
+    ReduceShiftColumn<false>(A, blockIdx.x * 64u + threadIdx.x, t);
+    if(A.hostOut && blockIdx.x < kShiftOutGroups)
+    {
+        __threadfence_system();
+        if(threadIdx.x == 0)
+        {
+            const uint32_t c = __hip_atomic_fetch_add(A.outArrived, 1u, __ATOMIC_ACQ_REL, __HIP_MEMORY_SCOPE_AGENT);
+            if(c + 1u == A.outTarget)
+            {
+                __threadfence_system();
+                __hip_atomic_store(A.hostFlag, A.hostSeq, __ATOMIC_RELEASE, __HIP_MEMORY_SCOPE_SYSTEM);
+            }
+        }
+    }
+}
+
+__global__ void __launch_bounds__(256) __attribute__((amdgpu_num_vgpr(48))) ReduceShiftResidentKernel(DeviceLayout L, ReduceShiftCall A, ResidentReduceArgs R,
+    uint32_t readShare0, PostResident PR)
+{
+    __shared__ float slice[4][64];
+    const uint32_t tid = threadIdx.x;
+    __builtin_amdgcn_s_setprio(3);
+    if(tid == 0)
+    {
+        if(!PostWaitCounter(R.counters + 16u * (kRcArrive0 + R.set), R.arriveTarget, 4, blockIdx.x == 0 ? R.counters + 16u * kRcWaitArrive : nullptr))
+            __hip_atomic_store(R.hostFlags + 16u * kRhError, 2u, __ATOMIC_RELAXED, __HIP_MEMORY_SCOPE_SYSTEM);
+    }
+    __syncthreads();
+    auto mid = [&]()
+    {
+        asm volatile("s_waitcnt vmcnt(0)" ::: "memory");
+        __syncthreads();
+        if(tid == 0)
+        {
+            __hip_atomic_fetch_add(R.counters + 16u * kRcRedRead, blockIdx.x == 0 ? readShare0 : 1u, __ATOMIC_RELAXED, __HIP_MEMORY_SCOPE_AGENT);
+            if(!PostWaitCounter(R.counters + 16u * kRcPostDone, R.postDoneTarget, 4, blockIdx.x == 0 ? R.counters + 16u * kRcWaitPost : nullptr))
+                __hip_atomic_store(R.hostFlags + 16u * kRhError, 3u, __ATOMIC_RELAXED, __HIP_MEMORY_SCOPE_SYSTEM);
+        }
+        __syncthreads();
+    };
+    const float t = AccumReduceBlock<true, true>(L, A.carry, slice, blockIdx.x, __builtin_amdgcn_readfirstlane(tid >> 6), tid & 63u, mid);
+    if(tid >= 64) return;
+    ReduceShiftColumn<true>(A, blockIdx.x * 64u + tid, t);
+    if(A.hostOut) __threadfence_system();
+    asm volatile("s_waitcnt vmcnt(0) lgkmcnt(0)" ::: "memory");
+    if(tid == 0)
+    {
+        const uint32_t c = __hip_atomic_fetch_add(PR.postDone, 1u, A.hostOut ? __ATOMIC_ACQ_REL : __ATOMIC_RELAXED, __HIP_MEMORY_SCOPE_AGENT);
+        if(c + 1u == PR.postDoneTarget)
+        {
+            if(A.hostOut)
+            {
+                __threadfence_system();
+                __hip_atomic_store(A.hostFlag, A.hostSeq, __ATOMIC_RELEASE, __HIP_MEMORY_SCOPE_SYSTEM);
+            }
+            __hip_atomic_store(PR.progress, PR.progressValue, __ATOMIC_RELAXED, __HIP_MEMORY_SCOPE_SYSTEM);
+        }
+    }
+}
+
 __global__ void OALGPU_SINGLE_DS_OPS __launch_bounds__(64) __attribute__((amdgpu_num_vgpr(48))) PostResidentKernel(const float *__restrict__ in, uint32_t nch,
     const SplitterState *__restrict__ spIn, SplitterState *__restrict__ spOut, const float *__restrict__ hfscales,
     const float *__restrict__ chanCoeffs, uint32_t taps, const float *__restrict__ accIn, float *__restrict__ carryOut,
@@ -420,6 +504,21 @@
     hipExtLaunchKernelGGL(ReducePostFusedKernel, dim3(A.nReduce + p.nch + kPostFrames / kFusedFrames), dim3(256), 0, s, nullptr, p.evDone, 0u, L, A);
 }
 
+uint32_t ReduceShiftGroups() { return kShiftGroups; }
+uint32_t ReduceShiftOutGroups() { return kShiftOutGroups; }
+void LaunchReduceShift(hipStream_t s, const DeviceLayout &L, const ReduceShiftCall &p, hipEvent_t evDone)
+{
+    hipExtLaunchKernelGGL(ReduceShiftKernel, dim3(kShiftGroups), dim3(256), 0, s, nullptr, evDone, 0u, L, p);
+}
+
+void LaunchReduceShiftResident(hipStream_t s, const DeviceLayout &L, const ReduceShiftCall &p, uint32_t *counters, uint32_t *hostFlags, uint32_t set,
+    uint32_t arriveTarget, uint32_t postDoneBefore, uint32_t redGroups, uint32_t postDoneTarget, uint32_t progressValue, hipEvent_t evDone)
+{
+    const PostResident PR{counters + 16u * kRcPostDone, postDoneTarget, hostFlags + 16u * kRhProgress, progressValue, hostFlags + 16u * kRhError, counters};
+    hipExtLaunchKernelGGL(ReduceShiftResidentKernel, dim3(kShiftGroups), dim3(256), 0, s, nullptr, evDone, 0u, L, p,
+        ResidentReduceArgs{counters, hostFlags, set, arriveTarget, postDoneBefore}, redGroups - (kShiftGroups - 1u), PR);
+}
+
 void LaunchPostDirectHrtfFast(hipStream_t s, float *left, float *right, const float *in, uint32_t nch, float *accum,
     SplitterState *splitters, const float *hfscales, const float *chanCoeffs, uint32_t irsize, uint32_t n, float *temp, hipEvent_t evDone)
 {
diff --git a/openal-soft_amd/oalgpu/__init__.py b/openal-soft_amd/oalgpu/__init__.py
--- a/openal-soft_amd/oalgpu/__init__.py
+++ b/openal-soft_amd/oalgpu/__init__.py
@@ -78,6 +78,8 @@
 CTX_SLICE_LINES = 128
 CTX_WAVE_PAIRS = 256
 CTX_ROW_SLICES = 512
+CTX_FULL_POST = 1024
+POST_NONE, POST_FULL, POST_SHORT = 0, 1, 2
 
 
 class VoiceDesc(C.Structure):
@@ -963,6 +965,12 @@
         check(lib.oalgpu_bus_device_ptr(self.h, C.byref(p), C.byref(n), C.byref(s)))
         return p.value, n.value, s.value
 
+    def last_post_path(self):
+        lib.oalgpu_last_post_path.argtypes = [C.c_void_p, C.POINTER(C.c_int)]
+        p = C.c_int(0)
+        check(lib.oalgpu_last_post_path(self.h, C.byref(p)))
+        return p.value
+
     def voice_kernel_name(self):
         lib.oalgpu_voice_kernel_name.restype = C.c_char_p
         lib.oalgpu_voice_kernel_name.argtypes = [C.c_void_p]
```

Result: slower. 106.4 million (-2.3%).
